# thegenemyers/FASTGA

Measured on NVIDIA H100. Metric: Gbp aligned/sec (genome x genome), higher is better.
Workload: dtype int32

## Files before the change

fastga_b200/csrc/api.cu:

```cuda
#include "common.cuh"
#include "handles.h"
#include <vector>
#include <algorithm>
#include <string.h>
#include <chrono>

typedef unsigned long long u64;

static inline long long now_us()
{ return std::chrono::duration_cast<std::chrono::microseconds>(std::chrono::steady_clock::now().time_since_epoch()).count(); }

extern "C" {
int fgb_kmer_sort_range_device(void *d_a, void *d_b, long long n, unsigned plo, unsigned phi,
                               void *d_tmp, long long tmp_bytes, int *result_in_b, void *stream);
int fgb_sort128_bits_device(void *d_a, void *d_b, long long n, int bit_lo, int bit_hi,
                            void *d_tmp, long long tmp_bytes, int *result_in_b, void *stream);
int fgb_sort128_device(void *d_a, void *d_b, long long n, int byte_lo, int byte_hi,
                       void *d_tmp, long long tmp_bytes, int *result_in_b, void *stream);
long long fgb_sort128_tmp_bytes(long long n);
int fgb_sort_seeds64_device(void *d_a, void *d_b, long long n, int bit_lo, int bit_hi,
                            void *d_tmp, long long tmp_bytes, unsigned long long *d_flag, void *stream);
int fgb_stage_genome_device(const void *d_bps, const long long *d_boff, const long long *d_clen,
                            const long long *d_woff, int ncontig, long long total_words,
                            void *d_seq, void *d_rseq, void *stream);
int fgb_syncmer_count_device(const void *d_seq, const long long *d_clen, const long long *d_woff,
                             const int *d_crank, const int *d_tile_contig, const int *d_tile_start,
                             int ntiles, unsigned *d_tile_count, unsigned long long *d_buck1024,
                             unsigned long long *d_total, void *d_tmp, long long tmp_bytes,
                             unsigned plo, unsigned phi, void *stream);
int fgb_syncmer_emit_device(const void *d_seq, const long long *d_clen, const long long *d_woff,
                            const int *d_crank, const int *d_tile_contig, const int *d_tile_start,
                            int ntiles, unsigned *d_tile_offset, void *d_records, unsigned plo,
                            unsigned phi, void *stream);
int fgb_kix_index_device(const void *d_tab, long long n, unsigned *d_pstart, unsigned char *d_adj, void *stream);
int fgb_ktab_export_device(const void *d_tab, long long n, int pbytes, int cbytes,
                           const long long *d_part_first, int nparts, void *d_out, void *stream);
int fgb_ktab_import_device(const void *d_ent, long long n, int pbytes, int cbytes,
                           const long long *d_index, void *d_tab, void *stream);
int fgb_sc_tile();
int fgb_owner_count_device(const void *d_seeds, long long n, int p_ic, int ic_bits, const int *d_owner, int nrc,
                           int world, unsigned long long *d_cnt, void *stream);
int fgb_owner_scatter_device(const void *d_seeds, long long n, int p_ic, int ic_bits, const int *d_owner, int nrc,
                             int world, unsigned long long *d_base, void *d_out, void *stream);
int fgb_kmer_bins_device(const void *d_tab, long long n, int binshift, unsigned *d_bins, void *stream);
int fgb_self_merge_device(const void *d_T, long long n, const unsigned *d_pstart, int freq,
                          int anti_bits, int band_bits, int jc_bits, int ic_bits,
                          long long amxpos, void *d_seeds, long long capacity,
                          unsigned long long *d_counters, unsigned long long *h_nseeds,
                          unsigned long long *h_sumlen, void *stream);
int fgb_forward_view_device(const void *d_T, long long n, void *d_out, long long *h_nfwd, void *stream);
int fgb_merge_device(const void *d_T1, long long n1, const void *d_T2, long long n2, const unsigned *d_pstart2,
                     const unsigned char *d_adj2, int freq, int anti_bits, int band_bits, int jc_bits, int ic_bits,
                     long long amxpos, long long bmxpos, void *d_seeds, long long capacity,
                     unsigned long long *d_counters, unsigned long long *h_nseeds,
                     unsigned long long *h_sumlen, void *stream);
}

static fgb_timings g_timings;

struct stage_timer
{ cudaEvent_t a, b; cudaStream_t st; float *dst;
  stage_timer(float *d, cudaStream_t s) : st(s), dst(d)
    { cudaEventCreate(&a); cudaEventCreate(&b); cudaEventRecord(a,st); }
  ~stage_timer()
    { cudaEventRecord(b,st); cudaEventSynchronize(b);
      float ms = 0; cudaEventElapsedTime(&ms,a,b); *dst += ms;
      cudaEventDestroy(a); cudaEventDestroy(b);
    }
};

void fgb_timing_add(int which, float ms)
{ if (which == 0) g_timings.triples_ms += ms;
  else if (which == 1) { g_timings.extend_ms += ms; g_timings.extend_launches += 1; }
  else if (which == 3) { g_timings.merge_ms += ms; g_timings.merge_launches += 1; }
  else g_timings.d2h_ms += ms;
}

void fgb_count_launch(int n) { g_timings.launches += n; }


#include <map>
#include <unordered_map>
#include <mutex>

static std::multimap<size_t,void *> g_free;
static std::unordered_map<void *,size_t> g_live;
static std::mutex g_mem_lock;

static size_t size_class(size_t b)
{ if (b < 4096) return 4096;
  size_t p = 4096;
  while (p < b) p <<= 1;
  size_t step = p >> 4;
  return ((b + step - 1) / step) * step;
}

cudaError_t fgb_dmalloc(void **p, size_t bytes, cudaStream_t st)
{ (void) st;
  size_t c = size_class(bytes);
  std::lock_guard<std::mutex> g(g_mem_lock);
  auto it = g_free.lower_bound(c);
  if (it != g_free.end() && it->first <= c + (c >> 2))
    { *p = it->second;
      g_live[*p] = it->first;
      g_free.erase(it);
      return cudaSuccess;
    }
  cudaError_t e = cudaMalloc(p,c);
  if (e != cudaSuccess)
    { cudaGetLastError();
      for (auto &kv : g_free) cudaFree(kv.second);
      g_free.clear();
      e = cudaMalloc(p,c);
      if (e != cudaSuccess) return e;
    }
  g_live[*p] = c;
  return cudaSuccess;
}

void fgb_dfree(void *p, cudaStream_t st)
{ (void) st;
  if (p == NULL) return;
  std::lock_guard<std::mutex> g(g_mem_lock);
  auto it = g_live.find(p);
  if (it == g_live.end()) { cudaFree(p); return; }
  g_free.insert(std::make_pair(it->second,p));
  g_live.erase(it);
}

extern "C" void fgb_release_cache()
{ std::lock_guard<std::mutex> g(g_mem_lock);
  for (auto &kv : g_free) cudaFree(kv.second);
  g_free.clear();
}

extern "C" void fgb_timings_reset() { memset(&g_timings,0,sizeof(g_timings)); }
extern "C" void fgb_timings_get(fgb_timings *out) { *out = g_timings; }


static const long long *g_sort_len;
static int LSORT(const void *l, const void *r)
{ int x = *((const int *) l), y = *((const int *) r);
  return (int) (g_sort_len[y] - g_sort_len[x]);
}

extern "C" int fgb_genome_create(const unsigned char *bps, long long bps_bytes, int ncontig,
                                 const long long *clen, const long long *boff, int want_revcomp,
                                 fgb_genome **out, void *stream)
{ cudaStream_t st = (cudaStream_t) stream;
  if (ncontig <= 0 || ncontig > 0x7fff) return FGB_ERR_LIMIT;
  fgb_genome *g = new fgb_genome();
  g->ncontig = ncontig;
  g->clen.assign(clen,clen+ncontig);
  g->boff.assign(boff,boff+ncontig);
  g->woff.resize(ncontig+1);
  g->seqtot = 0; g->maxlen = 0;
  long long w = 2;
  for (int c = 0; c < ncontig; c++)
    { if (clen[c] >= 0x7fffffffll) { delete g; return FGB_ERR_LIMIT; }
      g->woff[c] = w;
      w += ((clen[c] + 31) >> 5) + 2;
      w = (w + 1) & ~1ll;
      g->seqtot += clen[c];
      if (clen[c] > g->maxlen) g->maxlen = clen[c];
    }
  g->woff[ncontig] = w;
  g->total_words = w;

  g->perm.resize(ncontig); g->crank.resize(ncontig);
  for (int c = 0; c < ncontig; c++) g->perm[c] = c;
  g_sort_len = clen;
  qsort(g->perm.data(),ncontig,sizeof(int),LSORT);
  for (int c = 0; c < ncontig; c++) g->crank[g->perm[c]] = c;

  unsigned char *d_bps = NULL;
  long long *d_boff = NULL;
  CUDA_TRY(fgb_dmalloc((void **) &d_bps,bps_bytes + 16,st));
  CUDA_TRY(fgb_dmalloc((void **) &d_boff,sizeof(long long)*ncontig,st));
  CUDA_TRY(fgb_dmalloc((void **) &g->d_clen,sizeof(long long)*ncontig,st));
  CUDA_TRY(fgb_dmalloc((void **) &g->d_woff,sizeof(long long)*(ncontig+1),st));
  CUDA_TRY(fgb_dmalloc((void **) &g->d_crank,sizeof(int)*ncontig,st));
  CUDA_TRY(fgb_dmalloc((void **) &g->d_perm,sizeof(int)*ncontig,st));
  CUDA_TRY(fgb_dmalloc((void **) &g->d_seq,sizeof(u64)*(w + 1024),st));
  if (want_revcomp) CUDA_TRY(fgb_dmalloc((void **) &g->d_rseq,sizeof(u64)*(w + 1024),st));
  { stage_timer t(&g_timings.h2d_ms,st);
    CUDA_TRY(cudaMemcpyAsync(d_bps,bps,bps_bytes,cudaMemcpyHostToDevice,st));
    CUDA_TRY(cudaMemcpyAsync(d_boff,boff,sizeof(long long)*ncontig,cudaMemcpyHostToDevice,st));
    CUDA_TRY(cudaMemcpyAsync(g->d_clen,clen,sizeof(long long)*ncontig,cudaMemcpyHostToDevice,st));
    CUDA_TRY(cudaMemcpyAsync(g->d_woff,g->woff.data(),sizeof(long long)*(ncontig+1),cudaMemcpyHostToDevice,st));
    CUDA_TRY(cudaMemcpyAsync(g->d_crank,g->crank.data(),sizeof(int)*ncontig,cudaMemcpyHostToDevice,st));
    CUDA_TRY(cudaMemcpyAsync(g->d_perm,g->perm.data(),sizeof(int)*ncontig,cudaMemcpyHostToDevice,st));
  }
  g->h2d_bytes = bps_bytes + (long long) ncontig*(3*8+2*4) + 8;
  int rc;
  { stage_timer t(&g_timings.stage_ms,st);
    rc = fgb_stage_genome_device(d_bps,d_boff,g->d_clen,g->d_woff,ncontig,w,g->d_seq,g->d_rseq,st);
  }
  CUDA_TRY(cudaStreamSynchronize(st));
  fgb_dfree(d_bps,st); fgb_dfree(d_boff,st);
  if (rc) { delete g; return rc; }
  *out = g;
  return FGB_OK;
}

extern "C" void fgb_genome_free(fgb_genome *g)
{ cudaStream_t st = 0;
  if (!g) return;
  fgb_dfree(g->d_clen,st); fgb_dfree(g->d_woff,st); fgb_dfree(g->d_crank,st); fgb_dfree(g->d_perm,st);
  fgb_dfree(g->d_seq,st); fgb_dfree(g->d_rseq,st);
  delete g;
}

extern "C" int fgb_genome_perm(const fgb_genome *g, int *perm_out)
{ memcpy(perm_out,g->perm.data(),sizeof(int)*g->ncontig); return FGB_OK; }

extern "C" int fgb_genome_download(const fgb_genome *g, int rev, unsigned long long *words,
                                   long long *woff_out)
{ const u64 *src = rev ? g->d_rseq : g->d_seq;
  if (src == NULL) return FGB_ERR_ARG;
  CUDA_TRY(cudaMemcpy(words,src,sizeof(u64)*g->total_words,cudaMemcpyDeviceToHost));
  memcpy(woff_out,g->woff.data(),sizeof(long long)*(g->ncontig+1));
  return FGB_OK;
}
extern "C" long long fgb_genome_words(const fgb_genome *g) { return g->total_words; }


extern "C" void fgb_gix_free(fgb_gix *x)
{ cudaStream_t st = 0;
  if (!x) return;
  fgb_dfree(x->d_tab,st); fgb_dfree(x->d_pstart,st); fgb_dfree(x->d_adj,st);
  delete x;
}

static void gix_bytes(const fgb_genome *g, fgb_gix *x)
{ long long cum;
  x->post_bytes = 0;
  for (cum = 1; cum < g->maxlen; cum *= 256) x->post_bytes += 1;
  x->cont_bytes = 0;
  for (cum = 1; cum < 2ll*g->ncontig; cum *= 256) x->cont_bytes += 1;
}


#define GIX_FWD_ONLY 0x80000000u
#define GIX_NO_INDEX 0x40000000u

static int gix_build_range(const fgb_genome *g, unsigned plo, unsigned phi, fgb_gix **out, void *stream);

struct gix_scope
{ fgb_gix *x;
  explicit gix_scope(fgb_gix *p) : x(p) {}
  fgb_gix *release() { fgb_gix *p = x; x = NULL; return p; }
  ~gix_scope() { if (x != NULL) fgb_gix_free(x); }
};
struct blk_scope
{ std::vector<void **> slots;
  template<class T> void own(T *&p) { slots.push_back((void **) &p); }
  ~blk_scope() { for (void **s : slots) if (*s != NULL) { fgb_dfree(*s,0); *s = NULL; } }
};

extern "C" int fgb_gix_build(const fgb_genome *g, fgb_gix **out, void *stream)
{ return gix_build_range(g,0u,1u << 24,out,stream); }

extern "C" int fgb_gix_build_forward(const fgb_genome *g, fgb_gix **out, void *stream)
{ return gix_build_range(g,0u,(1u << 24) | GIX_FWD_ONLY,out,stream); }

extern "C" int fgb_gix_build_range(const fgb_genome *g, unsigned plo, unsigned phi, fgb_gix **out, void *stream)
{ if (plo > phi || phi > (1u << 24)) return FGB_ERR_ARG;
  return gix_build_range(g,plo,phi,out,stream);
}

static int gix_scan(const fgb_genome *g, const unsigned char *mask, unsigned plo, unsigned phi_flags,
                    rec128 **d_recs, long long *n_out, long long *nrev, unsigned long long *buck1024, cudaStream_t st)
{ int T = fgb_sc_tile();
  std::vector<int> tc, ts;
  for (int c = 0; c < g->ncontig; c++)
    if (g->clen[c] >= 12 && g->boff[c] >= 0 && (mask == NULL || mask[c]))
      for (long long t0 = 0; t0 + 12 <= g->clen[c]; t0 += T)
        { tc.push_back(c); ts.push_back((int) t0); }
  int ntiles = (int) tc.size();
  int *d_tc = NULL, *d_ts = NULL; unsigned *d_cnt = NULL;
  u64 *d_buck = NULL, *d_total = NULL; void *d_tmp = NULL;
  rec128 *d_a = NULL;
  long long tmpb = fgb_dev_scan_tmp_bytes(ntiles);
  int rc = FGB_OK;
  u64 total = 0, rdropped = 0;
#define GS_TRY(call) do { if ((call) != cudaSuccess) { rc = FGB_ERR_CUDA; goto done; } } while (0)
  GS_TRY(fgb_dmalloc((void **) &d_tc,sizeof(int)*(ntiles+1),st));
  GS_TRY(fgb_dmalloc((void **) &d_ts,sizeof(int)*(ntiles+1),st));
  GS_TRY(fgb_dmalloc((void **) &d_cnt,sizeof(unsigned)*(ntiles+1),st));
  GS_TRY(fgb_dmalloc((void **) &d_buck,8*1025,st));
  GS_TRY(fgb_dmalloc((void **) &d_total,8,st));
  GS_TRY(fgb_dmalloc((void **) &d_tmp,tmpb,st));
  GS_TRY(cudaMemcpyAsync(d_tc,tc.data(),sizeof(int)*ntiles,cudaMemcpyHostToDevice,st));
  GS_TRY(cudaMemcpyAsync(d_ts,ts.data(),sizeof(int)*ntiles,cudaMemcpyHostToDevice,st));
  { stage_timer t(&g_timings.scan_ms,st);
    rc = fgb_syncmer_count_device(g->d_seq,g->d_clen,g->d_woff,g->d_crank,d_tc,d_ts,ntiles,d_cnt,
                                  d_buck,d_total,d_tmp,tmpb,plo,phi_flags,st);
    if (rc) goto done;
    GS_TRY(cudaMemcpyAsync(&total,d_total,8,cudaMemcpyDeviceToHost,st));
    if (buck1024) GS_TRY(cudaMemcpyAsync(buck1024,d_buck,8*1024,cudaMemcpyDeviceToHost,st));
    GS_TRY(cudaMemcpyAsync(&rdropped,d_buck + 1024,8,cudaMemcpyDeviceToHost,st));
    GS_TRY(cudaStreamSynchronize(st));
  }
  if (total >= 0xfffffff0ull) { rc = FGB_ERR_LIMIT; goto done; }
  GS_TRY(fgb_dmalloc((void **) &d_a,sizeof(rec128)*(total+1),st));
  { stage_timer t(&g_timings.scan_ms,st);
    rc = fgb_syncmer_emit_device(g->d_seq,g->d_clen,g->d_woff,g->d_crank,d_tc,d_ts,ntiles,d_cnt,d_a,plo,phi_flags,st);
  }
  if (rc == FGB_OK && cudaStreamSynchronize(st) != cudaSuccess) rc = FGB_ERR_CUDA;
done:
#undef GS_TRY
  fgb_dfree(d_tc,st); fgb_dfree(d_ts,st); fgb_dfree(d_cnt,st); fgb_dfree(d_buck,st); fgb_dfree(d_total,st); fgb_dfree(d_tmp,st);
  if (rc) { fgb_dfree(d_a,st); return rc; }
  *d_recs = d_a; *n_out = (long long) total; *nrev = (long long) rdropped;
  return FGB_OK;
}

static int gix_finish(fgb_gix *x, rec128 *d_a, long long n, unsigned plo, unsigned phi, cudaStream_t st, bool index = true)
{ rec128 *d_b = NULL; void *d_stmp = NULL;
  long long stmpb = fgb_sort128_tmp_bytes(n);
  int rc = FGB_OK, inb = 0;
  x->n = n;
  if (fgb_dmalloc((void **) &d_b,sizeof(rec128)*(n+1),st) != cudaSuccess ||
      fgb_dmalloc((void **) &d_stmp,stmpb,st) != cudaSuccess ||
      (index && fgb_dmalloc((void **) &x->d_pstart,sizeof(unsigned)*((1<<24)+1+8),st) != cudaSuccess) ||
      (index && fgb_dmalloc((void **) &x->d_adj,(size_t) n + 32,st) != cudaSuccess))
    rc = FGB_ERR_CUDA;
  if (!rc)
    { stage_timer t(&g_timings.ksort_ms,st);
      rc = fgb_kmer_sort_range_device(d_a,d_b,n,plo,phi,d_stmp,stmpb,&inb,st);
    }
  if (!rc)
    { x->d_tab = inb ? d_b : d_a;
      if (inb) d_b = NULL; else d_a = NULL;
      if (index)
        { stage_timer t(&g_timings.index_ms,st);
          rc = fgb_kix_index_device(x->d_tab,n,x->d_pstart,x->d_adj,st);
        }
    }
  if (!rc && cudaStreamSynchronize(st) != cudaSuccess) rc = FGB_ERR_CUDA;
  fgb_dfree(d_a,st); fgb_dfree(d_b,st); fgb_dfree(d_stmp,st);
  return rc;
}

static int gix_build_range(const fgb_genome *g, unsigned plo, unsigned phi_flags, fgb_gix **out, void *stream)
{ cudaStream_t st = (cudaStream_t) stream;
  const bool index = !(phi_flags & GIX_NO_INDEX);
  phi_flags &= ~GIX_NO_INDEX;
  const unsigned phi = phi_flags & ~GIX_FWD_ONLY;
  fgb_gix *x = new fgb_gix();
  gix_bytes(g,x);
  x->ncontig = g->ncontig;
  x->fwd_only = (phi_flags & GIX_FWD_ONLY) ? 1 : 0;
  rec128 *d_a = NULL; long long n = 0, nrev = 0;
  int rc = gix_scan(g,NULL,plo,phi_flags,&d_a,&n,&nrev,x->buck1024,st);
  if (!rc) { x->n_both = n + nrev; rc = gix_finish(x,d_a,n,plo,phi,st,index); }
  if (rc) { fgb_gix_free(x); return rc; }
  *out = x;
  return FGB_OK;
}


extern "C" int fgb_device_alloc(long long bytes, void **out, void *stream)
{ CUDA_TRY(fgb_dmalloc(out,(size_t) (bytes > 0 ? bytes : 16),(cudaStream_t) stream)); return FGB_OK; }
extern "C" void fgb_device_free(void *p) { fgb_dfree(p,0); }

extern "C" int fgb_kmers_scan(const fgb_genome *g, const unsigned char *mask, int fwd_only,
                              void **d_recs, long long *n, void *stream)
{ rec128 *d = NULL; long long nrev = 0;
  int rc = gix_scan(g,mask,0u,(1u << 24) | (fwd_only ? GIX_FWD_ONLY : 0u),&d,n,&nrev,NULL,(cudaStream_t) stream);
  if (rc) return rc;
  *d_recs = d;
  return FGB_OK;
}

extern "C" int fgb_records_group_by_top_byte(void *d_recs, long long n, void *d_out, long long *bounds257,
                                             void *stream)
{ cudaStream_t st = (cudaStream_t) stream;
  for (int b = 0; b <= 256; b++) bounds257[b] = 0;
  if (n <= 0) return FGB_OK;
  void *d_tmp = NULL; unsigned *d_bins = NULL;
  long long tmpb = fgb_sort128_tmp_bytes(n);
  int rc = FGB_OK, inb = 0;
  std::vector<unsigned> bins(65537);
  if (fgb_dmalloc(&d_tmp,tmpb,st) != cudaSuccess || fgb_dmalloc((void **) &d_bins,sizeof(unsigned)*65537,st) != cudaSuccess)
    rc = FGB_ERR_CUDA;
  if (!rc) rc = fgb_sort128_device(d_recs,d_out,n,15,16,d_tmp,tmpb,&inb,st);
  if (!rc && !inb && cudaMemcpyAsync(d_out,d_recs,sizeof(rec128)*n,cudaMemcpyDeviceToDevice,st) != cudaSuccess) rc = FGB_ERR_CUDA;
  if (!rc) rc = fgb_kmer_bins_device(d_out,n,56,d_bins,st);
  if (!rc && (cudaMemcpyAsync(bins.data(),d_bins,sizeof(unsigned)*65537,cudaMemcpyDeviceToHost,st) != cudaSuccess ||
              cudaStreamSynchronize(st) != cudaSuccess)) rc = FGB_ERR_CUDA;
  fgb_dfree(d_tmp,st); fgb_dfree(d_bins,st);
  if (rc) return rc;
  for (int b = 0; b <= 256; b++) bounds257[b] = bins[b];
  return FGB_OK;
}

extern "C" int fgb_gix_from_records(const void *d_recs, long long n, unsigned plo, unsigned phi, int fwd_only,
                                    int post_bytes, int cont_bytes, int ncontig, fgb_gix **out, void *stream)
{ cudaStream_t st = (cudaStream_t) stream;
  if (n < 0 || n >= 0xfffffff0ll || plo >= phi || phi > (1u << 24)) return FGB_ERR_ARG;
  fgb_gix *x = new fgb_gix();
  x->n_both = n; x->post_bytes = post_bytes; x->cont_bytes = cont_bytes; x->ncontig = ncontig;
  x->fwd_only = fwd_only ? 1 : 0;
  rec128 *d_a = NULL;
  int rc = FGB_OK;
  if (fgb_dmalloc((void **) &d_a,sizeof(rec128)*(n+1),st) != cudaSuccess) rc = FGB_ERR_CUDA;
  if (!rc && n > 0 && cudaMemcpyAsync(d_a,d_recs,sizeof(rec128)*n,cudaMemcpyDeviceToDevice,st) != cudaSuccess) rc = FGB_ERR_CUDA;
  if (!rc) rc = gix_finish(x,d_a,n,plo,phi,st); else fgb_dfree(d_a,st);
  if (rc) { fgb_gix_free(x); return rc; }
  *out = x;
  return FGB_OK;
}

extern "C" long long fgb_gix_size(const fgb_gix *x) { return x->n; }

extern "C" int fgb_gix_copy_table(const fgb_gix *x, void *d_dst, void *stream)
{ CUDA_TRY(cudaMemcpyAsync(d_dst,x->d_tab,sizeof(rec128)*x->n,cudaMemcpyDeviceToDevice,(cudaStream_t) stream));
  CUDA_TRY(cudaStreamSynchronize((cudaStream_t) stream));
  return FGB_OK;
}

extern "C" int fgb_gix_from_device(const void *d_tab, long long n, int post_bytes, int cont_bytes,
                                   int ncontig, fgb_gix **out, void *stream)
{ cudaStream_t st = (cudaStream_t) stream;
  if (n >= 0xfffffff0ll) return FGB_ERR_LIMIT;
  fgb_gix *x = new fgb_gix();
  gix_scope own(x);
  x->n = n; x->n_both = n; x->post_bytes = post_bytes; x->cont_bytes = cont_bytes; x->ncontig = ncontig;
  CUDA_TRY(fgb_dmalloc((void **) &x->d_tab,sizeof(rec128)*(n+1),st));
  CUDA_TRY(fgb_dmalloc((void **) &x->d_pstart,sizeof(unsigned)*((1<<24)+1+8),st));
  CUDA_TRY(fgb_dmalloc((void **) &x->d_adj,(size_t) x->n + 32,st));
  CUDA_TRY(cudaMemcpyAsync(x->d_tab,d_tab,sizeof(rec128)*n,cudaMemcpyDeviceToDevice,st));
  int rc;
  { stage_timer t(&g_timings.index_ms,st);
    rc = fgb_kix_index_device(x->d_tab,n,x->d_pstart,x->d_adj,st);
  }
  CUDA_TRY(cudaStreamSynchronize(st));
  if (rc) return rc;
  *out = own.release();
  return FGB_OK;
}
extern "C" int fgb_gix_post_bytes(const fgb_gix *x) { return x->post_bytes; }
extern "C" int fgb_gix_cont_bytes(const fgb_gix *x) { return x->cont_bytes; }

extern "C" int fgb_gix_download(const fgb_gix *x, void *tab , unsigned *pstart ,
                                unsigned long long *buck1024)
{ if (tab) CUDA_TRY(cudaMemcpy(tab,x->d_tab,sizeof(rec128)*x->n,cudaMemcpyDeviceToHost));
  if (pstart) CUDA_TRY(cudaMemcpy(pstart,x->d_pstart,sizeof(unsigned)*((1<<24)+1),cudaMemcpyDeviceToHost));
  if (buck1024) memcpy(buck1024,x->buck1024,8*1024);
  return FGB_OK;
}

extern "C" int fgb_gix_upload(const void *tab, long long n, int post_bytes, int cont_bytes,
                              int ncontig, fgb_gix **out, void *stream)
{ cudaStream_t st = (cudaStream_t) stream;
  if (n >= 0xfffffff0ll) return FGB_ERR_LIMIT;
  fgb_gix *x = new fgb_gix();
  gix_scope own(x);
  x->n = n; x->n_both = n; x->post_bytes = post_bytes; x->cont_bytes = cont_bytes; x->ncontig = ncontig;
  CUDA_TRY(fgb_dmalloc((void **) &x->d_tab,sizeof(rec128)*(n+1),st));
  CUDA_TRY(fgb_dmalloc((void **) &x->d_pstart,sizeof(unsigned)*((1<<24)+1+8),st));
  CUDA_TRY(fgb_dmalloc((void **) &x->d_adj,(size_t) x->n + 32,st));
  CUDA_TRY(cudaMemcpyAsync(x->d_tab,tab,sizeof(rec128)*n,cudaMemcpyHostToDevice,st));
  int rc = fgb_kix_index_device(x->d_tab,n,x->d_pstart,x->d_adj,st);
  CUDA_TRY(cudaStreamSynchronize(st));
  if (rc) return rc;
  *out = own.release();
  return FGB_OK;
}

extern "C" int fgb_gix_import_ktab(const unsigned char *entries, long long n, int post_bytes,
                                   int cont_bytes, const long long *index, int ncontig,
                                   fgb_gix **out, void *stream)
{ cudaStream_t st = (cudaStream_t) stream;
  if (n >= 0xfffffff0ll || post_bytes > 4 || cont_bytes > 2) return FGB_ERR_LIMIT;
  fgb_gix *x = new fgb_gix();
  gix_scope own(x);
  x->n = n; x->n_both = n; x->post_bytes = post_bytes; x->cont_bytes = cont_bytes; x->ncontig = ncontig;
  long long E = 9 + post_bytes + cont_bytes;
  unsigned char *d_ent = NULL; long long *d_index = NULL;
  blk_scope B; B.own(d_ent); B.own(d_index);
  CUDA_TRY(fgb_dmalloc((void **) &d_ent,E*n + 16,st));
  CUDA_TRY(fgb_dmalloc((void **) &d_index,8ll<<24,st));
  CUDA_TRY(fgb_dmalloc((void **) &x->d_tab,sizeof(rec128)*(n+1),st));
  CUDA_TRY(fgb_dmalloc((void **) &x->d_pstart,sizeof(unsigned)*((1<<24)+1+8),st));
  CUDA_TRY(fgb_dmalloc((void **) &x->d_adj,(size_t) x->n + 32,st));
  CUDA_TRY(cudaMemcpyAsync(d_ent,entries,E*n,cudaMemcpyHostToDevice,st));
  CUDA_TRY(cudaMemcpyAsync(d_index,index,8ll<<24,cudaMemcpyHostToDevice,st));
  int rc = fgb_ktab_import_device(d_ent,n,post_bytes,cont_bytes,d_index,x->d_tab,st);
  if (!rc) rc = fgb_kix_index_device(x->d_tab,n,x->d_pstart,x->d_adj,st);
  CUDA_TRY(cudaStreamSynchronize(st));
  if (rc) return rc;
  *out = own.release();
  return FGB_OK;
}

extern "C" int fgb_gix_export_ktab(const fgb_gix *x, const long long *part_first, int nparts,
                                   unsigned char *out, void *stream)
{ cudaStream_t st = (cudaStream_t) stream;
  long long E = 9 + x->post_bytes + x->cont_bytes;
  unsigned char *d_out = NULL; long long *d_pf = NULL;
  blk_scope B; B.own(d_out); B.own(d_pf);
  CUDA_TRY(fgb_dmalloc((void **) &d_out,E*x->n + 16,st));
  CUDA_TRY(fgb_dmalloc((void **) &d_pf,8*(nparts+1),st));
  CUDA_TRY(cudaMemcpyAsync(d_pf,part_first,8*nparts,cudaMemcpyHostToDevice,st));
  int rc = fgb_ktab_export_device(x->d_tab,x->n,x->post_bytes,x->cont_bytes,d_pf,nparts,d_out,st);
  if (!rc) CUDA_TRY(cudaMemcpyAsync(out,d_out,E*x->n,cudaMemcpyDeviceToHost,st));
  CUDA_TRY(cudaStreamSynchronize(st));
  return rc;
}


static int bitlen(long long v) { int b = 0; while (v > 0) { b += 1; v >>= 1; } return b; }

extern "C" void fgb_seeds_free(fgb_seeds *s)
{ cudaStream_t st = 0;
  if (!s) return;
  fgb_dfree(s->d_rec,st);
  delete s;
}

static int seeds_find_impl(const fgb_gix *x1, const fgb_gix *x2, long long amxpos,
                           long long bmxpos, int freq, bool self, fgb_seeds **out, void *stream);

extern "C" int fgb_seeds_find(const fgb_gix *x1, const fgb_gix *x2, long long amxpos,
                              long long bmxpos, int freq, fgb_seeds **out, void *stream)
{ return seeds_find_impl(x1,x2,amxpos,bmxpos,freq,false,out,stream); }

extern "C" int fgb_seeds_find_self(const fgb_gix *x, long long amxpos, int freq, fgb_seeds **out, void *stream)
{ return seeds_find_impl(x,x,amxpos,amxpos,freq,true,out,stream); }

struct seed_bits { int anti, band, jc, ic, key; };

static int seed_layout_of(const fgb_gix *x1, const fgb_gix *x2, long long amxpos, long long bmxpos, seed_bits *L)
{ L->anti = bitlen(amxpos + bmxpos);
  L->band = L->anti > 6 ? L->anti - 6 : 1;
  L->jc   = bitlen(x2->ncontig > 1 ? x2->ncontig-1 : 1);
  L->ic   = bitlen(x1->ncontig > 1 ? x1->ncontig-1 : 1);
  L->key  = 12 + L->anti + L->band + L->jc + L->ic + 1;
  return L->key > 128 ? FGB_ERR_LIMIT : FGB_OK;
}

static int seeds_merge_impl(const fgb_gix *x1, const fgb_gix *x2, long long amxpos, long long bmxpos, int freq,
                            bool self, const seed_bits &L, rec128 **d_out, long long *nseeds_out,
                            long long *sumlen_out, long long *n1m_out, cudaStream_t st)
{ if (self && x1->fwd_only) return FGB_ERR_ARG;
  u64 *d_counters = NULL; rec128 *d_fwd = NULL, *d_a = NULL;
  int rc = FGB_OK;
  u64 nseeds = 0, sumlen = 0;
  const rec128 *t1 = x1->d_tab; long long n1 = x1->n;
#define SF_TRY(call) do { if ((call) != cudaSuccess) { rc = FGB_ERR_CUDA; goto done; } } while (0)
  SF_TRY(fgb_dmalloc((void **) &d_counters,16,st));
  if (!self && !x1->fwd_only && n1 > 0)
    { SF_TRY(fgb_dmalloc((void **) &d_fwd,sizeof(rec128)*(n1+1),st));
      if ((rc = fgb_forward_view_device(x1->d_tab,n1,d_fwd,&n1,st))) goto done;
      t1 = d_fwd;
    }
  { long long cap = (self ? 2*x1->n : 2*n1 + (n1 >> 1)) + 1024;
    for (int attempt = 0; ; attempt++)
      { SF_TRY(fgb_dmalloc((void **) &d_a,sizeof(rec128)*(cap+1),st));
        if (self)
          rc = fgb_self_merge_device(x1->d_tab,x1->n,x1->d_pstart,freq,L.anti,L.band,L.jc,L.ic,amxpos,
                                     d_a,cap,d_counters,&nseeds,&sumlen,st);
        else
          rc = fgb_merge_device(t1,n1,x2->d_tab,x2->n,x2->d_pstart,x2->d_adj,freq,L.anti,L.band,L.jc,L.ic,
                                amxpos,bmxpos,d_a,cap,d_counters,&nseeds,&sumlen,st);
        if (rc == FGB_OK) break;
        fgb_dfree(d_a,st); d_a = NULL;
        if (rc != FGB_ERR_OVERFLOW || attempt > 0) goto done;
        cap = (long long) nseeds + 1024;
        g_timings.merge_ms = 0; g_timings.merge_launches = 0;
      }
  }
  if (nseeds >= 0xfffffff0ull) rc = FGB_ERR_LIMIT;
done:
#undef SF_TRY
  fgb_dfree(d_counters,st); fgb_dfree(d_fwd,st);
  if (rc) { fgb_dfree(d_a,st); return rc; }
  *d_out = d_a; *nseeds_out = (long long) nseeds; *sumlen_out = (long long) sumlen; *n1m_out = n1;
  return FGB_OK;
}

static int seeds_sort_impl(rec128 *d_a, long long n, const seed_bits &L, long long amxpos, long long bmxpos,
                           bool self, long long sumlen, long long n1m, fgb_seeds **out, cudaStream_t st)
{ rec128 *d_b = NULL; void *d_tmp = NULL;
  fgb_seeds *s = new fgb_seeds();
  s->self_mode = self ? 1 : 0;
  s->anti_bits = L.anti; s->band_bits = L.band; s->jc_bits = L.jc; s->ic_bits = L.ic;
  s->amxpos = amxpos; s->bmxpos = bmxpos;
  s->n = n; s->sumlen = sumlen; s->n1_merged = n1m;
  long long tmpb = fgb_sort128_tmp_bytes(n);
  int rc = FGB_OK, inb = 0;
  const char *wide_env = getenv("FGB_SEED_SORT_WIDE");
  const bool narrow = L.key <= 64 && !(wide_env != NULL && atoi(wide_env) != 0);
  u64 hiflag = 0, *d_hiflag = NULL;
  if (fgb_dmalloc((void **) &d_b,sizeof(rec128)*(n+1),st) != cudaSuccess ||
      fgb_dmalloc((void **) &d_tmp,tmpb + 8,st) != cudaSuccess) rc = FGB_ERR_CUDA;
  if (!rc)
    { stage_timer t(&g_timings.ssort_ms,st);
      if (narrow)
        { d_hiflag = (u64 *) ((char *) d_tmp + tmpb);
          rc = fgb_sort_seeds64_device(d_a,d_b,n,6,L.key,d_tmp,tmpb,d_hiflag,st);
        }
      else
        rc = fgb_sort128_bits_device(d_a,d_b,n,6,L.key,d_tmp,tmpb,&inb,st);
    }
  if (!rc && d_hiflag && cudaMemcpyAsync(&hiflag,d_hiflag,8,cudaMemcpyDeviceToHost,st) != cudaSuccess) rc = FGB_ERR_CUDA;
  if (!rc && cudaStreamSynchronize(st) != cudaSuccess) rc = FGB_ERR_CUDA;
  if (!rc && hiflag) rc = FGB_ERR_ARG;
  if (!rc)
    { s->d_rec = inb ? d_b : d_a;
      if (inb) d_b = NULL; else d_a = NULL;
    }
  fgb_dfree(d_a,st); fgb_dfree(d_b,st); fgb_dfree(d_tmp,st);
  if (rc) { delete s; return rc; }
  *out = s;
  return FGB_OK;
}

static int seeds_find_impl(const fgb_gix *x1, const fgb_gix *x2, long long amxpos,
                           long long bmxpos, int freq, bool self, fgb_seeds **out, void *stream)
{ cudaStream_t st = (cudaStream_t) stream;
  seed_bits L;
  int rc = seed_layout_of(x1,x2,amxpos,bmxpos,&L);
  if (rc) return rc;
  rec128 *d_a = NULL; long long n = 0, sumlen = 0, n1m = 0;
  if ((rc = seeds_merge_impl(x1,x2,amxpos,bmxpos,freq,self,L,&d_a,&n,&sumlen,&n1m,st))) return rc;
  return seeds_sort_impl(d_a,n,L,amxpos,bmxpos,self,sumlen,n1m,out,st);
}


extern "C" int fgb_seeds_merge(const fgb_gix *x1, const fgb_gix *x2, long long amxpos, long long bmxpos, int freq,
                               void **d_seeds, long long *n, int *bits, long long *info, void *stream)
{ seed_bits L;
  int rc = seed_layout_of(x1,x2,amxpos,bmxpos,&L);
  if (rc) return rc;
  rec128 *d_a = NULL; long long sumlen = 0, n1m = 0;
  if ((rc = seeds_merge_impl(x1,x2,amxpos,bmxpos,freq,false,L,&d_a,n,&sumlen,&n1m,(cudaStream_t) stream))) return rc;
  *d_seeds = d_a;
  bits[0] = L.anti; bits[1] = L.band; bits[2] = L.jc; bits[3] = L.ic;
  if (info) { info[0] = sumlen; info[1] = n1m; }
  return FGB_OK;
}

extern "C" int fgb_seeds_group_by_owner(const void *d_seeds, long long n, const int *bits, const int *owner,
                                        int nrank_contigs, int world, void *d_out, long long *bounds,
                                        void *stream)
{ cudaStream_t st = (cudaStream_t) stream;
  if (world < 1 || world > 64) return FGB_ERR_ARG;
  for (int w = 0; w <= world; w++) bounds[w] = 0;
  if (n <= 0) return FGB_OK;
  int *d_owner = NULL; u64 *d_cnt = NULL;
  int rc = FGB_OK;
  u64 cnt[64], base[65];
  const int p_ic = 12 + bits[0] + bits[1] + bits[2];
  if (fgb_dmalloc((void **) &d_owner,sizeof(int)*(size_t) nrank_contigs,st) != cudaSuccess ||
      fgb_dmalloc((void **) &d_cnt,8*64*2,st) != cudaSuccess) rc = FGB_ERR_CUDA;
  if (!rc && (cudaMemcpyAsync(d_owner,owner,sizeof(int)*(size_t) nrank_contigs,cudaMemcpyHostToDevice,st) != cudaSuccess ||
              cudaMemsetAsync(d_cnt,0,8*64*2,st) != cudaSuccess)) rc = FGB_ERR_CUDA;
  if (!rc) rc = fgb_owner_count_device(d_seeds,n,p_ic,bits[3],d_owner,nrank_contigs,world,d_cnt,st);
  if (!rc && (cudaMemcpyAsync(cnt,d_cnt,8*64,cudaMemcpyDeviceToHost,st) != cudaSuccess ||
              cudaStreamSynchronize(st) != cudaSuccess)) rc = FGB_ERR_CUDA;
  if (!rc)
    { base[0] = 0;
      for (int w = 0; w < world; w++) base[w+1] = base[w] + cnt[w];
      if (cudaMemcpyAsync(d_cnt + 64,base,8*64,cudaMemcpyHostToDevice,st) != cudaSuccess) rc = FGB_ERR_CUDA;
    }
  if (!rc) rc = fgb_owner_scatter_device(d_seeds,n,p_ic,bits[3],d_owner,nrank_contigs,world,d_cnt + 64,d_out,st);
  if (!rc && cudaStreamSynchronize(st) != cudaSuccess) rc = FGB_ERR_CUDA;
  fgb_dfree(d_owner,st); fgb_dfree(d_cnt,st);
  if (rc) return rc;
  for (int w = 0; w <= world; w++) bounds[w] = (long long) base[w];
  return FGB_OK;
}

extern "C" int fgb_records_group_by_owner(const void *d_recs, long long n, const int *owner256, int world,
                                          void *d_out, long long *bounds, void *stream)
{ cudaStream_t st = (cudaStream_t) stream;
  if (world < 1 || world > 64) return FGB_ERR_ARG;
  for (int w = 0; w <= world; w++) bounds[w] = 0;
  if (n <= 0) return FGB_OK;
  int *d_owner = NULL; u64 *d_cnt = NULL;
  int rc = FGB_OK;
  u64 cnt[64], base[65];
  if (fgb_dmalloc((void **) &d_owner,sizeof(int)*256,st) != cudaSuccess ||
      fgb_dmalloc((void **) &d_cnt,8*64*2,st) != cudaSuccess) rc = FGB_ERR_CUDA;
  if (!rc && (cudaMemcpyAsync(d_owner,owner256,sizeof(int)*256,cudaMemcpyHostToDevice,st) != cudaSuccess ||
              cudaMemsetAsync(d_cnt,0,8*64*2,st) != cudaSuccess)) rc = FGB_ERR_CUDA;
  if (!rc) rc = fgb_owner_count_device(d_recs,n,120,8,d_owner,256,world,d_cnt,st);
  if (!rc && (cudaMemcpyAsync(cnt,d_cnt,8*64,cudaMemcpyDeviceToHost,st) != cudaSuccess ||
              cudaStreamSynchronize(st) != cudaSuccess)) rc = FGB_ERR_CUDA;
  if (!rc)
    { base[0] = 0;
      for (int w = 0; w < world; w++) base[w+1] = base[w] + cnt[w];
      if (cudaMemcpyAsync(d_cnt + 64,base,8*64,cudaMemcpyHostToDevice,st) != cudaSuccess) rc = FGB_ERR_CUDA;
    }
  if (!rc) rc = fgb_owner_scatter_device(d_recs,n,120,8,d_owner,256,world,d_cnt + 64,d_out,st);
  if (!rc && cudaStreamSynchronize(st) != cudaSuccess) rc = FGB_ERR_CUDA;
  fgb_dfree(d_owner,st); fgb_dfree(d_cnt,st);
  if (rc) return rc;
  for (int w = 0; w <= world; w++) bounds[w] = (long long) base[w];
  return FGB_OK;
}

extern "C" int fgb_seeds_from_records(const void *d_recs, long long n, const int *bits, long long amxpos,
                                      long long bmxpos, long long sumlen, fgb_seeds **out, void *stream)
{ cudaStream_t st = (cudaStream_t) stream;
  if (n < 0 || n >= 0xfffffff0ll) return FGB_ERR_LIMIT;
  seed_bits L;
  L.anti = bits[0]; L.band = bits[1]; L.jc = bits[2]; L.ic = bits[3];
  L.key = 12 + L.anti + L.band + L.jc + L.ic + 1;
  if (L.key > 128) return FGB_ERR_LIMIT;
  rec128 *d_a = NULL;
  CUDA_TRY(fgb_dmalloc((void **) &d_a,sizeof(rec128)*(n+1),st));
  if (n > 0 && cudaMemcpyAsync(d_a,d_recs,sizeof(rec128)*n,cudaMemcpyDeviceToDevice,st) != cudaSuccess)
    { fgb_dfree(d_a,st); return FGB_ERR_CUDA; }
  return seeds_sort_impl(d_a,n,L,amxpos,bmxpos,false,sumlen,0,out,st);
}

extern "C" long long fgb_seeds_size(const fgb_seeds *s) { return s->n; }
extern "C" long long fgb_seeds_sumlen(const fgb_seeds *s) { return s->sumlen; }
extern "C" int fgb_seeds_layout(const fgb_seeds *s, int *bits )
{ bits[0] = s->anti_bits; bits[1] = s->band_bits; bits[2] = s->jc_bits; bits[3] = s->ic_bits; return FGB_OK; }
extern "C" int fgb_seeds_download(const fgb_seeds *s, void *rec)
{ CUDA_TRY(cudaMemcpy(rec,s->d_rec,sizeof(rec128)*s->n,cudaMemcpyDeviceToHost)); return FGB_OK; }

extern "C" int fgb_sort128_host(void *recs, long long n, int byte_lo, int byte_hi, void *stream)
{ cudaStream_t st = (cudaStream_t) stream;
  rec128 *d_a = NULL, *d_b = NULL; void *d_tmp = NULL;
  long long tmpb = fgb_sort128_tmp_bytes(n);
  CUDA_TRY(fgb_dmalloc((void **) &d_a,sizeof(rec128)*(n+1),st));
  CUDA_TRY(fgb_dmalloc((void **) &d_b,sizeof(rec128)*(n+1),st));
  CUDA_TRY(fgb_dmalloc((void **) &d_tmp,tmpb,st));
  CUDA_TRY(cudaMemcpyAsync(d_a,recs,sizeof(rec128)*n,cudaMemcpyHostToDevice,st));
  int inb = 0;
  int rc = fgb_sort128_device(d_a,d_b,n,byte_lo,byte_hi,d_tmp,tmpb,&inb,st);
  if (!rc) CUDA_TRY(cudaMemcpyAsync(recs,inb ? d_b : d_a,sizeof(rec128)*n,cudaMemcpyDeviceToHost,st));
  CUDA_TRY(cudaStreamSynchronize(st));
  fgb_dfree(d_a,st); fgb_dfree(d_b,st); fgb_dfree(d_tmp,st);
  return rc;
}

extern "C" int fgb_device_ready()
{ int n = 0;
  if (cudaGetDeviceCount(&n) != cudaSuccess || n == 0) return 0;
  return 1;
}


struct fgb_overlaps;
struct fgb_alns;
extern "C" {
int fgb_extend(const fgb_seeds *S, const fgb_genome *A, const fgb_genome *B, int chain_break,
               int chain_min, int align_min, double align_rate, const short *tables, int ave_path,
               int tspace, fgb_overlaps **out, void *stream);
int fgb_align_spec(double ave_corr, const float *freq, short *tables, int *ave_path);
void fgb_overlaps_free(fgb_overlaps *o);
long long fgb_overlaps_bytes(const fgb_overlaps *o);
void fgb_overlaps_counters(const fgb_overlaps *o, unsigned long long *out);
int fgb_filter(const fgb_overlaps *O, const int *perm1, const int *perm2, int jc_bits, int ic_bits,
               int do_filter, fgb_alns **out);
}

struct fgb_run_stats
{ long long nkmers1, nkmers2, nseeds, sumlen, nhits, nla, nwaves, ncells, nraw, h2d_bytes, d2h_bytes,
            nseg, nwork, warp_cycles, wave_cycles, extract_cycles,
            us_gix, us_seeds, us_extend, us_filter, nkmers1_fwd,
            slow_cycles, slow_waves, paired_waves, pairings; };

extern "C" int fgb_align_tables(const fgb_genome *A, const fgb_genome *B, const fgb_gix *x1,
                                const fgb_gix *x2, const float *freqA,
                                int freq, int chain_break, int chain_min, int align_min,
                                double align_rate, fgb_alns **out, fgb_run_stats *stats, void *stream);

static int align_tables_impl(const fgb_genome *A, const fgb_genome *B, fgb_gix *x1, fgb_gix *x2, bool own,
                             const float *freqA, int freq, int chain_break, int chain_min, int align_min,
                             double align_rate, fgb_alns **out, fgb_run_stats *stats, void *stream);

extern "C" int fgb_align_resident(const fgb_genome *A, const fgb_genome *B, const float *freqA,
                                  int freq, int chain_break, int chain_min, int align_min,
                                  double align_rate, fgb_alns **out, fgb_run_stats *stats, void *stream)
{ fgb_gix *x1 = NULL, *x2 = NULL;
  int rc;
  long long t0 = now_us();
  if ((rc = gix_build_range(A,0u,(1u << 24) | GIX_FWD_ONLY | GIX_NO_INDEX,&x1,stream))) return rc;
  if ((rc = fgb_gix_build(B,&x2,stream))) { fgb_gix_free(x1); return rc; }
  long long t1 = now_us();
  rc = align_tables_impl(A,B,x1,x2,true,freqA,freq,chain_break,chain_min,align_min,align_rate,out,stats,stream);
  if (stats) stats->us_gix = t1 - t0;
  return rc;
}

extern "C" int fgb_align_tables(const fgb_genome *A, const fgb_genome *B, const fgb_gix *x1,
                                const fgb_gix *x2, const float *freqA,
                                int freq, int chain_break, int chain_min, int align_min,
                                double align_rate, fgb_alns **out, fgb_run_stats *stats, void *stream)
{ return align_tables_impl(A,B,(fgb_gix *) x1,(fgb_gix *) x2,false,freqA,freq,chain_break,chain_min,align_min,
                           align_rate,out,stats,stream);
}

static int align_tables_impl(const fgb_genome *A, const fgb_genome *B, fgb_gix *x1, fgb_gix *x2, bool own,
                             const float *freqA, int freq, int chain_break, int chain_min, int align_min,
                             double align_rate, fgb_alns **out, fgb_run_stats *stats, void *stream)
{ fgb_seeds *sd = NULL; fgb_overlaps *ov = NULL;
  int rc;
  long long t0 = now_us(), t1 = t0, t2, t3, t4;
  const long long n1 = x1->n_both, n2 = x2->n;
  { seed_bits L;
    rec128 *d_a = NULL; long long n = 0, sumlen = 0, n1m = 0;
    rc = seed_layout_of(x1,x2,A->maxlen,B->maxlen,&L);
    if (!rc) rc = seeds_merge_impl(x1,x2,A->maxlen,B->maxlen,freq,false,L,&d_a,&n,&sumlen,&n1m,(cudaStream_t) stream);
    if (own) { fgb_gix_free(x1); fgb_gix_free(x2); }
    if (!rc) rc = seeds_sort_impl(d_a,n,L,A->maxlen,B->maxlen,false,sumlen,n1m,&sd,(cudaStream_t) stream);
  }
  if (rc) return rc;
  const long long n1f = sd->n1_merged;
  t2 = now_us();
  short *tables = (short *) malloc(65536*sizeof(short));
  int ave = 0;
  fgb_align_spec(1.-align_rate,freqA,tables,&ave);
  rc = fgb_extend(sd,A,B,chain_break,chain_min,align_min,align_rate,tables,ave,100,&ov,stream);
  free(tables);
  t3 = now_us();
  long long nseeds = sd->n, sumlen = sd->sumlen;
  int jb = sd->jc_bits, ib = sd->ic_bits;
  fgb_seeds_free(sd);
  if (rc) return rc;
  rc = fgb_filter(ov,A->perm.data(),B->perm.data(),jb,ib,1,out);
  t4 = now_us();
  if (stats)
    { stats->us_gix = t1-t0; stats->us_seeds = t2-t1; stats->us_extend = t3-t2; stats->us_filter = t4-t3; unsigned long long c[16];
      fgb_overlaps_counters(ov,c);
      stats->nkmers1 = n1; stats->nkmers2 = n2; stats->nseeds = nseeds; stats->sumlen = sumlen;
      stats->nkmers1_fwd = n1f;
      stats->nhits = (long long) c[0]; stats->nla = (long long) c[1]; stats->nwaves = (long long) c[2];
      stats->ncells = (long long) c[3]; stats->nraw = 0;
      stats->nseg = (long long) c[5]; stats->nwork = (long long) c[6];
      stats->warp_cycles = (long long) c[8]; stats->wave_cycles = (long long) c[9];
      stats->extract_cycles = (long long) c[10];
      stats->slow_cycles = (long long) ((c[15] >> 40) << 12); stats->slow_waves = (long long) ((c[15] >> 16) & 0xffffff);
      stats->paired_waves = (long long) c[11]; stats->pairings = (long long) c[12];
      stats->h2d_bytes = A->h2d_bytes + B->h2d_bytes + 65536*2;
      stats->d2h_bytes = fgb_overlaps_bytes(ov) + 16 + 8*1024*2 + 64;
    }
  fgb_overlaps_free(ov);
  return rc;
}

extern "C" int fgb_fastga_self(const unsigned char *bps, long long nb, int nc, const long long *clen,
                               const long long *boff, const float *freq4,
                               int freq, int chain_break, int chain_min, int align_min, double align_rate,
                               fgb_alns **out, fgb_run_stats *stats, void *stream)
{ fgb_genome *A = NULL; fgb_gix *x = NULL; fgb_seeds *sd = NULL; fgb_overlaps *ov = NULL;
  int rc;
  if ((rc = fgb_genome_create(bps,nb,nc,clen,boff,1,&A,stream))) return rc;
  if ((rc = fgb_gix_build(A,&x,stream))) { fgb_genome_free(A); return rc; }
  rc = fgb_seeds_find_self(x,A->maxlen,freq,&sd,stream);
  long long n1 = x->n;
  fgb_gix_free(x);
  if (rc) { fgb_genome_free(A); return rc; }
  short *tables = (short *) malloc(65536*sizeof(short));
  int ave = 0;
  fgb_align_spec(1.-align_rate,freq4,tables,&ave);
  rc = fgb_extend(sd,A,A,chain_break,chain_min,align_min,align_rate,tables,ave,100,&ov,stream);
  free(tables);
  long long nseeds = sd->n, sumlen = sd->sumlen;
  int jb = sd->jc_bits, ib = sd->ic_bits;
  fgb_seeds_free(sd);
  if (rc) { fgb_genome_free(A); return rc; }
  rc = fgb_filter(ov,A->perm.data(),A->perm.data(),jb,ib,1,out);
  if (stats)
    { memset(stats,0,sizeof(*stats));
      unsigned long long c[16];
      fgb_overlaps_counters(ov,c);
      stats->nkmers1 = stats->nkmers2 = n1; stats->nseeds = nseeds; stats->sumlen = sumlen;
      stats->nhits = (long long) c[0]; stats->nla = (long long) c[1]; stats->nwaves = (long long) c[2];
      stats->ncells = (long long) c[3];
    }
  fgb_overlaps_free(ov);
  fgb_genome_free(A);
  return rc;
}

extern "C" int fgb_fastga(const unsigned char *bpsA, long long nbA, int ncA, const long long *clenA,
                          const long long *boffA, const float *freqA,
                          const unsigned char *bpsB, long long nbB, int ncB, const long long *clenB,
                          const long long *boffB,
                          int freq, int chain_break, int chain_min, int align_min, double align_rate,
                          fgb_alns **out, fgb_run_stats *stats, void *stream)
{ fgb_genome *A = NULL, *B = NULL;
  int rc;
  if ((rc = fgb_genome_create(bpsA,nbA,ncA,clenA,boffA,1,&A,stream))) return rc;
  if ((rc = fgb_genome_create(bpsB,nbB,ncB,clenB,boffB,0,&B,stream))) { fgb_genome_free(A); return rc; }
  rc = fgb_align_resident(A,B,freqA,freq,chain_break,chain_min,align_min,align_rate,out,stats,stream);
  fgb_genome_free(A); fgb_genome_free(B);
  return rc;
}
```

fastga_b200/csrc/gix.cu:

```cuda
#include "common.cuh"

static const unsigned char h_TMap[256] =
  { 0xff,0xd4,0xf5,0xfd,0xe4,0xad,0x21,0xa5,0xed,0x64,0xbf,0xa9,0xf3,0x70,0xd6,0xf0,
    0xca,0x89,0xcb,0xc9,0x82,0x9d,0x13,0x79,0x0a,0x0f,0x25,0x19,0x3e,0x47,0xa3,0xa8,
    0xf9,0x5e,0xe8,0xa1,0xb0,0x71,0x1d,0x8c,0xde,0x69,0xe7,0x7c,0x56,0x3f,0x90,0xa4,
    0xeb,0x45,0x59,0xf1,0x97,0x4c,0x08,0xa0,0xb8,0x4a,0x86,0xc8,0xcd,0x98,0x7d,0xfc,
    0xef,0x4d,0x83,0x7e,0xdc,0x66,0x2b,0x8e,0xe0,0xa7,0xd0,0xa2,0x88,0x5f,0x7f,0xd9,
    0x9b,0x78,0xd1,0x8b,0xc3,0x8f,0x2d,0xe6,0x18,0x27,0x2c,0x24,0x94,0xb7,0xce,0xbd,
    0x0d,0x04,0x1c,0x09,0x16,0x23,0x00,0x1e,0x1a,0x29,0x2e,0x15,0x01,0x10,0x2a,0x20,
    0xbe,0x31,0x43,0x58,0xc2,0xaa,0x1f,0xe5,0xc5,0x9e,0xcf,0xc6,0x68,0xb2,0x80,0xf4,
    0xf8,0x53,0xb6,0x93,0x76,0x37,0x11,0x40,0xda,0x51,0xba,0x46,0x42,0x30,0x60,0x6d,
    0x5c,0x39,0x9f,0x48,0x6c,0x62,0x28,0x67,0x06,0x12,0x26,0x0e,0x33,0x50,0xa6,0x63,
    0xdd,0x3b,0xab,0x4b,0x72,0x5b,0x22,0x6f,0xb4,0x61,0x92,0x99,0x36,0x38,0x65,0xac,
    0x4f,0x2f,0x32,0x44,0x54,0x3c,0x03,0x5d,0x73,0x3a,0x77,0x84,0x8d,0x4e,0x49,0xd2,
    0xfb,0x91,0x6a,0xcc,0x8a,0x35,0x02,0x55,0x7a,0x34,0x96,0x3d,0xd3,0x41,0x85,0xf2,
    0xb1,0x75,0xc4,0xb5,0xbb,0xb3,0x1b,0xd5,0x07,0x05,0x17,0x0b,0x7b,0xd7,0xdf,0xea,
    0xe3,0x57,0xc0,0x95,0x9c,0x6e,0x14,0xae,0xb9,0x6b,0xc1,0x81,0x87,0x74,0xd8,0xe2,
    0xec,0x52,0xbc,0xe9,0xe1,0xdb,0x0c,0xf7,0xaf,0x5a,0x9a,0xc7,0xfa,0xf6,0xee,0xfe };

__constant__ unsigned char c_TN[256];
__constant__ unsigned char c_TC[256];

static int tables_ready = 0;

static int init_tables()
{ if (tables_ready) return FGB_OK;
  unsigned char tn[256], tc[256];
  for (int x = 0; x < 256; x++)
    { int b0 = x & 3, b1 = (x>>2) & 3, b2 = (x>>4) & 3, b3 = (x>>6) & 3;
      int fwd = (b0<<6) | (b1<<4) | (b2<<2) | b3;
      int rc  = ((3-b3)<<6) | ((3-b2)<<4) | ((3-b1)<<2) | (3-b0);
      tn[x] = h_TMap[fwd];
      tc[x] = h_TMap[rc];
    }
  CUDA_TRY(cudaMemcpyToSymbol(c_TN,tn,256));
  CUDA_TRY(cudaMemcpyToSymbol(c_TC,tc,256));
  tables_ready = 1;
  return FGB_OK;
}

typedef unsigned long long u64;


static __device__ __forceinline__ u64 bases64(const u64 *__restrict__ w, long long nw, long long boff)
{ long long q = boff >> 5;
  int s = (int) (boff & 31) << 1;
  u64 a = (q >= 0 && q < nw) ? w[q] : 0ull;
  if (s == 0) return a;
  u64 b = (q+1 >= 0 && q+1 < nw) ? w[q+1] : 0ull;
  return (a >> s) | (b << (64-s));
}

static __device__ __forceinline__ u64 rev2(u64 x)
{ x = __brevll(x);
  return ((x & 0x5555555555555555ull) << 1) | ((x >> 1) & 0x5555555555555555ull);
}


__global__ void stage_contigs_kernel(const unsigned char *__restrict__ bps,
                                     const long long *__restrict__ boff,
                                     const long long *__restrict__ clen,
                                     const long long *__restrict__ woff, int ncontig,
                                     u64 *__restrict__ seq, long long total_words)
{ long long g = (long long) blockIdx.x * blockDim.x + threadIdx.x;
  if (g >= total_words) return;
  int lo = 0, hi = ncontig-1;
  while (lo < hi)
    { int m = (lo+hi+1) >> 1;
      if (woff[m] <= g) lo = m; else hi = m-1;
    }
  long long q = g - woff[lo];
  long long nbytes = (clen[lo]+3) >> 2;
  long long b0 = q*8;
  u64 v = 0;
  if (boff[lo] >= 0 && q >= 0)
    { const unsigned char *p = bps + boff[lo];
      for (int i = 0; i < 8; i++)
        if (b0+i < nbytes)
          v |= (u64) p[b0+i] << (8*i);
      long long lim = clen[lo] - q*32;
      if (lim < 32) v &= (lim <= 0) ? 0ull : ((1ull << (2*lim)) - 1);
    }
  seq[g] = v;
}

__global__ void revcomp_contigs_kernel(const u64 *__restrict__ seq, const long long *__restrict__ clen,
                                       const long long *__restrict__ woff, int ncontig,
                                       u64 *__restrict__ rseq, long long total_words)
{ long long g = (long long) blockIdx.x * blockDim.x + threadIdx.x;
  if (g >= total_words) return;
  int lo = 0, hi = ncontig-1;
  while (lo < hi)
    { int m = (lo+hi+1) >> 1;
      if (woff[m] <= g) lo = m; else hi = m-1;
    }
  long long q = g - woff[lo];
  long long L = clen[lo];
  long long nw = (lo+1 < ncontig ? woff[lo+1] : total_words) - woff[lo];
  if (q < 0) { rseq[g] = 0; return; }
  u64 e = bases64(seq + woff[lo],nw,L - 32 - 32*q);
  u64 v = ~rev2(e);
  long long lim = L - q*32;
  if (lim < 32) v &= (lim <= 0) ? 0ull : ((1ull << (2*lim)) - 1);
  rseq[g] = v;
}


#define SC_THREADS 256
#define SC_PPT     16
#define SC_TILE    (SC_THREADS*SC_PPT)
#define SC_WORDS   (SC_TILE/32 + 3)

static __device__ __forceinline__ u64 sm_bases64(const u64 *sw, int boff)
{ int q = boff >> 5, s = (boff & 31) << 1;
  u64 a = sw[q];
  if (s == 0) return a;
  return (a >> s) | (sw[q+1] << (64-s));
}


static __device__ __forceinline__ unsigned syncmer_mask(u64 E, const unsigned char *tn,
                                                        const unsigned char *tc)
{ unsigned hn[SC_PPT+8], hc[SC_PPT+8];
#pragma unroll
  for (int i = 0; i < SC_PPT+8; i++)
    { unsigned x = (unsigned) (E >> (2*i)) & 0xff;
      hn[i] = tn[x];
      hc[i] = tc[x];
    }
  unsigned mz[SC_PPT+4];
#pragma unroll
  for (int i = 0; i < SC_PPT+4; i++)
    { unsigned mn = (hn[i] << 8) | hn[i+4];
      unsigned mc = hc[i] | (hc[i+4] << 8);
      mz[i] = mn < mc ? mn : mc;
    }
  unsigned sel = 0;
#pragma unroll
  for (int i = 0; i < SC_PPT; i++)
    { unsigned m = min(min(min(mz[i],mz[i+1]),min(mz[i+2],mz[i+3])),mz[i+4]);
      if (mz[i] == m || mz[i+4] == m) sel |= 1u << i;
    }
  return sel;
}

template<int EMIT> __global__ void __launch_bounds__(SC_THREADS)
syncmer_kernel(const u64 *__restrict__ seq, const long long *__restrict__ clen,
               const long long *__restrict__ woff, const int *__restrict__ crank,
               const int *__restrict__ tile_contig, const int *__restrict__ tile_start,
               unsigned *__restrict__ tile_count,
               unsigned long long *__restrict__ buck1024,
               rec128 *__restrict__ out, unsigned plo, unsigned phi_flags)
{ __shared__ u64 sw[SC_WORDS+1];
  __shared__ unsigned char tn[256], tc[256];
  __shared__ unsigned wsum[SC_THREADS/32];
  __shared__ unsigned hist[1024];

  const unsigned phi = phi_flags & 0x7fffffffu;
  const bool fwd_only = (phi_flags >> 31) != 0;
  int tid = threadIdx.x;
  int c   = tile_contig[blockIdx.x];
  int t0  = tile_start[blockIdx.x];
  long long L  = clen[c];
  const u64 *w = seq + woff[c];
  long long nw = (L + 31) >> 5;

  tn[tid] = c_TN[tid];
  tc[tid] = c_TC[tid];
  if (EMIT == 0)
    for (int i = tid; i < 1024; i += SC_THREADS) hist[i] = 0;
  for (int i = tid; i < SC_WORDS+1; i += SC_THREADS)
    { long long gw = (t0 >> 5) - 1 + i;
      sw[i] = (gw >= 0 && gw < nw) ? w[gw] : 0ull;
    }
  __syncthreads();

  int p = t0 + tid*SC_PPT;
  int sb = 32 + tid*SC_PPT;
  unsigned sel = 0;
  if ((long long) p + 12 <= L)
    { sel = syncmer_mask(sm_bases64(sw,sb),tn,tc);
      long long lastok = L - 12 - p;
      if (lastok < SC_PPT-1) sel &= (2u << lastok) - 1;
    }

  unsigned fmask = sel, rmask = sel;
  { long long fl = L - 40 - p;
    if (fl < 0) fmask = 0; else if (fl < SC_PPT-1) fmask &= (2u << fl) - 1;
    int rl = 28 - p;
    if (rl > 0) rmask = (rl >= SC_PPT) ? 0 : (rmask & ~((1u << rl) - 1));
  }
  if (plo != 0 || phi != (1u << 24))
    { unsigned m = fmask | rmask;
      while (m)
        { int i = __ffs(m)-1;
          m &= m-1;
          if (fmask >> i & 1)
            { unsigned pf = (unsigned) (rev2(sm_bases64(sw,sb+i)) >> 40);
              if (pf < plo || pf >= phi) fmask &= ~(1u << i);
            }
          if (rmask >> i & 1)
            { u64 e0 = sm_bases64(sw,sb+i-28), e1 = sm_bases64(sw,sb+i+4) & 0xffffull;
              unsigned pr = (unsigned) ((~((e1 << 48) | (e0 >> 16))) >> 40);
              if (pr < plo || pr >= phi) rmask &= ~(1u << i);
            }
        }
    }
  unsigned rdropped = 0;
  if (fwd_only) { rdropped = __popc(rmask); rmask = 0; }
  unsigned cnt = __popc(fmask) + __popc(rmask);

  int lane = tid & 31, wp = tid >> 5;
  unsigned inc = cnt;
#pragma unroll
  for (int o = 1; o < 32; o <<= 1)
    { unsigned t = __shfl_up_sync(0xffffffffu,inc,o);
      if (lane >= o) inc += t;
    }
  if (lane == 31) wsum[wp] = inc;
  __syncthreads();
  unsigned pre = 0, tot = 0;
  for (int i = 0; i < SC_THREADS/32; i++)
    { if (i < wp) pre += wsum[i];
      tot += wsum[i];
    }

  if (EMIT == 0)
    {
      unsigned m = sel;
      while (m)
        { int i = __ffs(m)-1;
          m &= m-1;
          u64 f = sm_bases64(sw,sb+i);
          unsigned fb = (unsigned) (rev2(f) >> 54);
          u64 r = sm_bases64(sw,sb+i+7);
          unsigned rb = (unsigned) ((~r) & 0x3ff);
          unsigned rr = 0;
#pragma unroll
          for (int k = 0; k < 5; k++)
            rr |= ((rb >> (2*k)) & 3) << (2*k);
          atomicAdd(&hist[fb],1u);
          atomicAdd(&hist[rr],1u);
        }
      __syncthreads();
      for (int i = tid; i < 1024; i += SC_THREADS)
        if (hist[i]) atomicAdd(&buck1024[i],(unsigned long long) hist[i]);
      if (fwd_only)
        { rdropped = __reduce_add_sync(0xffffffffu,rdropped);
          if (lane == 0 && rdropped) atomicAdd(&buck1024[1024],(unsigned long long) rdropped);
        }
      if (tid == 0) tile_count[blockIdx.x] = tot;
      return;
    }

  long long o = (long long) tile_count[blockIdx.x] + pre + inc - cnt;
  unsigned cr = (unsigned) crank[c];
  unsigned m = fmask | rmask;
  while (m)
    { int i = __ffs(m)-1;
      m &= m-1;
      int j = p + i;
      if (fmask >> i & 1)
        { u64 e0 = sm_bases64(sw,sb+i);
          u64 e1 = sm_bases64(sw,sb+i+32);
          rec128 r;
          r.hi = rev2(e0);
          r.lo = (rev2(e1) & 0xffff000000000000ull) | ((u64) cr << 32) | (unsigned) j;
          st_rec(out + o,r);
          o += 1;
        }
      if (rmask >> i & 1)
        { u64 e0 = sm_bases64(sw,sb+i-28);
          u64 e1 = sm_bases64(sw,sb+i+4) & 0xffffull;
          rec128 r;
          r.hi = ~((e1 << 48) | (e0 >> 16));
          r.lo = ((~e0 & 0xffffull) << 48) | ((u64) (cr | 0x8000u) << 32) | (unsigned) (j+12);
          st_rec(out + o,r);
          o += 1;
        }
    }
}


__global__ void kix_index_kernel(const rec128 *__restrict__ tab, long long n,
                                 unsigned *__restrict__ pstart, unsigned char *__restrict__ adj)
{ long long i = (long long) blockIdx.x * blockDim.x + threadIdx.x;
  if (i > n) return;
  rec128 a, b;
  a.lo = a.hi = b.lo = b.hi = 0;
  if (i > 0) a = ld_rec(tab + i - 1);
  if (i < n) b = ld_rec(tab + i);
  if (i > 0 && i < n)
    { long long plo = (long long) KREC_PREFIX24(a.hi), phi = (long long) KREC_PREFIX24(b.hi);
      for (long long x = plo+1; x <= phi; x++)
        pstart[x] = (unsigned) i;
    }
  int l = 0;
  if (i > 0 && i < n)
    { unsigned long long x = a.hi ^ b.hi;
      if (x) l = __clzll(x) >> 1;
      else
        { unsigned y = (unsigned) ((a.lo ^ b.lo) >> 48);
          l = y ? 32 + ((__clz(y) - 16) >> 1) : 40;
        }
    }
  adj[i] = (unsigned char) l;
}

static __device__ __forceinline__ int krec_lcp(const rec128 &a, const rec128 &b)
{ u64 x = a.hi ^ b.hi;
  if (x) return __clzll(x) >> 1;
  unsigned y = (unsigned) ((a.lo ^ b.lo) >> 48);
  if (y) return 32 + ((__clz(y) - 16) >> 1);
  return 40;
}


__global__ void ktab_export_kernel(const rec128 *__restrict__ tab, long long n, int pbytes,
                                   int cbytes, const long long *__restrict__ part_first, int nparts,
                                   unsigned char *__restrict__ out)
{ long long i = (long long) blockIdx.x * blockDim.x + threadIdx.x;
  if (i >= n) return;
  rec128 r = tab[i];
  int lcp = 0;
  bool first = false;
  for (int p = 0; p < nparts; p++)
    if (part_first[p] == i) first = true;
  if (!first)
    lcp = krec_lcp(tab[i-1],r);
  int E = 9 + pbytes + cbytes;
  unsigned char *o = out + i*E;
  u64 suf = KREC_SUFFIX56(r);
  for (int k = 0; k < 7; k++)
    o[k] = (unsigned char) (suf >> (8*(6-k)));
  o[7] = 0;
  o[8] = (unsigned char) lcp;
  unsigned post = (unsigned) r.lo;
  for (int k = 0; k < pbytes; k++)
    o[9+k] = (unsigned char) (post >> (8*k));
  unsigned cs = (unsigned) (r.lo >> 32) & 0xffff;
  unsigned cv = (cs & 0x7fff) | ((cs >> 15) << (8*cbytes-1));
  for (int k = 0; k < cbytes; k++)
    o[9+pbytes+k] = (unsigned char) (cv >> (8*k));
}


__global__ void ktab_import_kernel(const unsigned char *__restrict__ ent, long long n, int pbytes,
                                   int cbytes, const long long *__restrict__ index ,
                                   rec128 *__restrict__ tab)
{ long long i = (long long) blockIdx.x * blockDim.x + threadIdx.x;
  if (i >= n) return;
  int lo = 0, hi = (1<<24)-1;
  while (lo < hi)
    { int m = (lo+hi) >> 1;
      if (index[m] > i) hi = m; else lo = m+1;
    }
  int E = 9 + pbytes + cbytes;
  const unsigned char *e = ent + i*E;
  u64 suf = 0;
  for (int k = 0; k < 7; k++)
    suf = (suf << 8) | e[k];
  unsigned post = 0;
  for (int k = 0; k < pbytes; k++)
    post |= (unsigned) e[9+k] << (8*k);
  unsigned cv = 0;
  for (int k = 0; k < cbytes; k++)
    cv |= (unsigned) e[9+pbytes+k] << (8*k);
  unsigned sign = cv >> (8*cbytes-1);
  unsigned cs = (cv & ((1u << (8*cbytes-1)) - 1)) | (sign << 15);
  rec128 r;
  r.hi = ((u64) lo << 40) | (suf >> 16);
  r.lo = ((suf & 0xffffull) << 48) | ((u64) cs << 32) | post;
  st_rec(tab + i,r);
}


extern "C" int fgb_sort128_device(void *d_a, void *d_b, long long n, int byte_lo, int byte_hi,
                                  void *d_tmp, long long tmp_bytes, int *result_in_b, void *stream);
extern "C" long long fgb_sort128_tmp_bytes(long long n);

extern "C" int fgb_stage_genome_device(const void *d_bps, const long long *d_boff,
                                       const long long *d_clen, const long long *d_woff,
                                       int ncontig, long long total_words, void *d_seq,
                                       void *d_rseq , void *stream)
{ cudaStream_t st = (cudaStream_t) stream;
  if (total_words <= 0) return FGB_OK;
  int nb = (int) ((total_words + 255) / 256);
  stage_contigs_kernel<<<nb,256,0,st>>>((const unsigned char *) d_bps,d_boff,d_clen,d_woff,ncontig,
                                        (u64 *) d_seq,total_words);
  if (d_rseq != NULL)
    revcomp_contigs_kernel<<<nb,256,0,st>>>((const u64 *) d_seq,d_clen,d_woff,ncontig,
                                            (u64 *) d_rseq,total_words);
  fgb_count_launch(d_rseq != NULL ? 2 : 1);
  CUDA_TRY(cudaGetLastError());
  return FGB_OK;
}


extern "C" int fgb_syncmer_count_device(const void *d_seq, const long long *d_clen,
                                        const long long *d_woff, const int *d_crank,
                                        const int *d_tile_contig, const int *d_tile_start, int ntiles,
                                        unsigned *d_tile_count, unsigned long long *d_buck1024,
                                        unsigned long long *d_total, void *d_tmp, long long tmp_bytes,
                                        unsigned plo, unsigned phi, void *stream)
{ cudaStream_t st = (cudaStream_t) stream;
  int rc = init_tables();
  if (rc) return rc;
  CUDA_TRY(cudaMemsetAsync(d_buck1024,0,1025*8,st));
  if (ntiles > 0)
    syncmer_kernel<0><<<ntiles,SC_THREADS,0,st>>>((const u64 *) d_seq,d_clen,d_woff,d_crank,
                                                   d_tile_contig,d_tile_start,d_tile_count,
                                                   d_buck1024,NULL,plo,phi);
  fgb_count_launch(1);
  CUDA_TRY(cudaGetLastError());
  return fgb_dev_exclusive_scan_u32(d_tile_count,ntiles,d_total,d_tmp,tmp_bytes,st);
}

extern "C" int fgb_syncmer_emit_device(const void *d_seq, const long long *d_clen,
                                       const long long *d_woff, const int *d_crank,
                                       const int *d_tile_contig, const int *d_tile_start, int ntiles,
                                       unsigned *d_tile_offset, void *d_records, unsigned plo,
                                       unsigned phi, void *stream)
{ cudaStream_t st = (cudaStream_t) stream;
  if (ntiles > 0)
    syncmer_kernel<1><<<ntiles,SC_THREADS,0,st>>>((const u64 *) d_seq,d_clen,d_woff,d_crank,
                                                   d_tile_contig,d_tile_start,d_tile_offset,
                                                   NULL,(rec128 *) d_records,plo,phi);
  fgb_count_launch(1);
  CUDA_TRY(cudaGetLastError());
  return FGB_OK;
}

__global__ void kix_ends_kernel(const rec128 *__restrict__ tab, long long n, unsigned *__restrict__ pstart)
{ long long x = (long long) blockIdx.x * blockDim.x + threadIdx.x;
  if (x > (1ll << 24)) return;
  if (n == 0) { pstart[x] = 0; return; }
  long long p0 = (long long) KREC_PREFIX24(tab[0].hi), pl = (long long) KREC_PREFIX24(tab[n-1].hi);
  if (x <= p0) pstart[x] = 0;
  else if (x > pl) pstart[x] = (unsigned) n;
}

extern "C" int fgb_kix_index_device(const void *d_tab, long long n, unsigned *d_pstart, unsigned char *d_adj,
                                    void *stream)
{ cudaStream_t st = (cudaStream_t) stream;
  int nb = (int) ((n + 1 + 255) / 256);
  CUDA_TRY(cudaMemsetAsync(d_adj + n,0,32,st));
  kix_index_kernel<<<nb,256,0,st>>>((const rec128 *) d_tab,n,d_pstart,d_adj);
  kix_ends_kernel<<<((1 << 24) + 256)/256,256,0,st>>>((const rec128 *) d_tab,n,d_pstart);
  fgb_count_launch(1);
  CUDA_TRY(cudaGetLastError());
  return FGB_OK;
}

extern "C" int fgb_ktab_export_device(const void *d_tab, long long n, int pbytes, int cbytes,
                                      const long long *d_part_first, int nparts, void *d_out,
                                      void *stream)
{ cudaStream_t st = (cudaStream_t) stream;
  if (n <= 0) return FGB_OK;
  int nb = (int) ((n + 255) / 256);
  ktab_export_kernel<<<nb,256,0,st>>>((const rec128 *) d_tab,n,pbytes,cbytes,d_part_first,nparts,
                                      (unsigned char *) d_out);
  CUDA_TRY(cudaGetLastError());
  return FGB_OK;
}

extern "C" int fgb_ktab_import_device(const void *d_ent, long long n, int pbytes, int cbytes,
                                      const long long *d_index, void *d_tab, void *stream)
{ cudaStream_t st = (cudaStream_t) stream;
  if (n <= 0) return FGB_OK;
  int nb = (int) ((n + 255) / 256);
  ktab_import_kernel<<<nb,256,0,st>>>((const unsigned char *) d_ent,n,pbytes,cbytes,d_index,
                                      (rec128 *) d_tab);
  CUDA_TRY(cudaGetLastError());
  return FGB_OK;
}

extern "C" int fgb_sc_tile() { return SC_TILE; }
```

fastga_b200/csrc/sort128.cu:

```cuda
#include "common.cuh"
#include <stdlib.h>
#include <vector>

#define SORT_THREADS 512
#ifndef SORT_ITEMS
#define SORT_ITEMS   8
#endif
#ifndef SORT_MINBLK
#define SORT_MINBLK  2
#endif
#define SORT_TILE    (SORT_THREADS*SORT_ITEMS)
#define SORT_WARPS   (SORT_THREADS/32)

static __device__ __forceinline__ unsigned warp_incl_scan(unsigned v, int lane)
{
#pragma unroll
  for (int o = 1; o < 32; o <<= 1)
    { unsigned t = __shfl_up_sync(0xffffffffu,v,o);
      if (lane >= o) v += t;
    }
  return v;
}



static __device__ __forceinline__ unsigned match_digit(unsigned d, bool valid)
{ unsigned peers = __ballot_sync(0xffffffffu,valid);
#pragma unroll
  for (int k = 0; k < 8; k++)
    { bool bit = (d >> k) & 1;
      unsigned bk = __ballot_sync(0xffffffffu,bit);
      peers &= bit ? bk : ~bk;
    }
  return peers;
}


#define ST_AGG  (1ull << 62)
#define ST_INC  (2ull << 62)
#define ST_MASK ((1ull << 62) - 1)

__global__ void __launch_bounds__(SORT_THREADS)
sort_ghist_kernel(const rec128 *__restrict__ in, long long n, int dsh , unsigned long long *__restrict__ ghist)
{ __shared__ unsigned h[256];
  int tid = threadIdx.x;
  if (tid < 256) h[tid] = 0;
  __syncthreads();
  const bool one = (dsh >= 64 || dsh <= 56);
  const unsigned long long *half = reinterpret_cast<const unsigned long long *>(in) + (dsh >= 64);
  const int sh = dsh & 63;
  for (long long tile0 = (long long) blockIdx.x * SORT_TILE; tile0 < n; tile0 += (long long) gridDim.x * SORT_TILE)
    {
#pragma unroll
      for (int it = 0; it < SORT_ITEMS; it++)
        { long long idx = tile0 + it*SORT_THREADS + tid;
          bool valid = idx < n;
          unsigned d = 0;
          if (valid) d = one ? (unsigned) ((half[2*idx] >> sh) & 0xff) : rec_dig(ld_rec(in + idx),dsh);
          unsigned peers = match_digit(d,valid);
          if (valid && (tid & 31) == __ffs(peers)-1) atomicAdd(&h[d],__popc(peers));
        }
    }
  __syncthreads();
  if (tid < 256 && h[tid]) atomicAdd(&ghist[tid],(unsigned long long) h[tid]);
}

__global__ void sort_bins_kernel(const unsigned long long *__restrict__ ghist, unsigned long long *__restrict__ binbase,
                                 unsigned long long *__restrict__ nexthist, unsigned *__restrict__ ticket)
{ __shared__ unsigned long long ws[8];
  int tid = threadIdx.x, lane = tid & 31, w = tid >> 5;
  unsigned long long v = ghist[tid], inc = v;
  for (int o = 1; o < 32; o <<= 1)
    { unsigned long long t = __shfl_up_sync(0xffffffffu,inc,o);
      if (lane >= o) inc += t;
    }
  if (lane == 31) ws[w] = inc;
  __syncthreads();
  unsigned long long pre = 0;
  for (int i = 0; i < w; i++) pre += ws[i];
  binbase[tid] = pre + inc - v;
  nexthist[tid] = 0;
  if (tid == 0) *ticket = 0;
}

__global__ void __launch_bounds__(SORT_THREADS,SORT_MINBLK)
sort_onesweep_kernel(const rec128 *__restrict__ in, rec128 *__restrict__ out, long long n, int byte ,
                     int next_byte , const unsigned long long *__restrict__ binbase,
                     unsigned long long *__restrict__ nexthist, unsigned long long *status ,
                     unsigned *__restrict__ ticket)
{ extern __shared__ __align__(16) unsigned char smem_raw[];
  rec128   *tile   = reinterpret_cast<rec128 *>(smem_raw);
  unsigned *wcount = reinterpret_cast<unsigned *>(tile + SORT_TILE);
  unsigned *bexcl  = wcount + SORT_WARPS*256;
  unsigned *nhist  = bexcl + 256;
  unsigned *wtot   = nhist + 256;
  unsigned long long *gbase = reinterpret_cast<unsigned long long *>(wtot + 8);
  __shared__ unsigned tile_s;
  __shared__ __align__(8) unsigned long long tbar;

  int tid = threadIdx.x, lane = tid & 31, w = tid >> 5;
  if (tid == 0)
    { unsigned t = atomicAdd(ticket,1u);
      tile_s = t;
      long long t0 = (long long) t * SORT_TILE, rm = n - t0;
      unsigned nb = (unsigned) (rm < SORT_TILE ? rm : SORT_TILE) * 16u;
      mbar_init(&tbar,1);
      tma_load_1d(tile,in + t0,nb,&tbar);
    }
  for (int i = tid; i < SORT_WARPS*256; i += SORT_THREADS) wcount[i] = 0;
  if (tid < 256) nhist[tid] = 0;
  __syncthreads();
  const unsigned tileid = tile_s;
  long long tile0 = (long long) tileid * SORT_TILE;
  long long rem = n - tile0;
  int cnt = rem < SORT_TILE ? (int) rem : SORT_TILE;

  rec128   r[SORT_ITEMS];
  unsigned rank[SORT_ITEMS];
  int base = w*(32*SORT_ITEMS);
  unsigned *myc = wcount + w*256;
  mbar_wait(&tbar,0);
#pragma unroll
  for (int it = 0; it < SORT_ITEMS; it++)
    { int idx = base + it*32 + lane;
      bool valid = idx < cnt;
      unsigned d = 0;
      if (valid)
        { r[it] = ld_rec(tile + idx);
          d = rec_dig(r[it],byte);
        }
      unsigned peers = match_digit(d,valid);
      int leader = valid ? __ffs(peers)-1 : lane;
      unsigned b = 0;
      if (valid && lane == leader)
        { b = myc[d];
          myc[d] = b + __popc(peers);
        }
      b = __shfl_sync(0xffffffffu,b,leader);
      rank[it] = b + __popc(peers & lanemask_lt());
      if (next_byte >= 0 && valid) atomicAdd(&nhist[rec_dig(r[it],next_byte)],1u);
      __syncwarp();
    }
  __syncthreads();

  unsigned c = 0, inc = 0;
  unsigned long long *mine = status + (unsigned long long) tileid*256 + tid;
  if (tid < 256)
    { unsigned sum = 0;
#pragma unroll
      for (int ww = 0; ww < SORT_WARPS; ww++)
        { unsigned t = wcount[ww*256+tid];
          wcount[ww*256+tid] = sum;
          sum += t;
        }
      c = sum;
      if (tileid == 0)
        atomicExch(mine,ST_INC | c);
      else
        atomicExch(mine,ST_AGG | c);
      inc = warp_incl_scan(c,lane);
      if (lane == 31) wtot[w] = inc;
    }
  __syncthreads();
  if (tid < 256)
    { unsigned pre = 0;
      for (int i = 0; i < w; i++) pre += wtot[i];
      bexcl[tid] = pre + inc - c;
    }
  __syncthreads();

#pragma unroll
  for (int it = 0; it < SORT_ITEMS; it++)
    { int idx = base + it*32 + lane;
      if (idx < cnt)
        { unsigned d = rec_dig(r[it],byte);
          st_rec(tile + (bexcl[d] + myc[d] + rank[it]),r[it]);
        }
    }
  if (tid < 256)
    {
      volatile unsigned long long *stt = status;
      unsigned long long excl = 0;
      for (long long t = (long long) tileid - 1; t >= 0; )
        { unsigned long long v[4];
#pragma unroll
          for (int q = 0; q < 4; q++)
            v[q] = (t - q >= 0) ? stt[(unsigned long long) (t - q)*256 + tid] : ST_INC;
          bool done = false;
#pragma unroll
          for (int q = 0; q < 4; q++)
            { if (done || (v[q] >> 62) == 0) break;
              excl += v[q] & ST_MASK;
              t -= 1;
              if (v[q] & ST_INC) done = true;
            }
          if (done) break;
        }
      if (tileid != 0) atomicExch(mine,ST_INC | (excl + c));
      gbase[tid] = binbase[tid] + excl - bexcl[tid];
      if (next_byte >= 0 && nhist[tid]) atomicAdd(&nexthist[tid],(unsigned long long) nhist[tid]);
    }
  __syncthreads();

  for (int p = tid; p < cnt; p += SORT_THREADS)
    { rec128 v = ld_rec(tile + p);
      unsigned d = rec_dig(v,byte);
      st_rec(out + (gbase[d] + p),v);
    }
}

static const size_t ONESWEEP_SMEM = SORT_TILE*sizeof(rec128) + (SORT_WARPS*256 + 256 + 256 + 8)*sizeof(unsigned)
                                    + 256*sizeof(unsigned long long);

extern "C" long long fgb_sort128_tmp_bytes(long long n)
{ long long ntiles = (n + SORT_TILE - 1) / SORT_TILE;
  if (ntiles < 1) ntiles = 1;
  return 256*ntiles*8 + (3*256 + 16)*8;
}


extern "C" int fgb_sort128_bits_device(void *d_a, void *d_b, long long n, int bit_lo, int bit_hi,
                                       void *d_tmp, long long tmp_bytes, int *result_in_b, void *stream)
{ cudaStream_t st = (cudaStream_t) stream;
  if (n < 0 || bit_lo < 0 || bit_hi > 128 || bit_lo > bit_hi) return FGB_ERR_ARG;
  if (n >= 0xffffffffll) return FGB_ERR_LIMIT;
  *result_in_b = 0;
  if (n <= 1 || bit_lo == bit_hi) return FGB_OK;
  if (tmp_bytes < fgb_sort128_tmp_bytes(n)) return FGB_ERR_ARG;

  int ntiles = (int) ((n + SORT_TILE - 1) / SORT_TILE);
  unsigned long long *status = (unsigned long long *) d_tmp;
  unsigned long long *hist[2] = { status + 256ull*ntiles, status + 256ull*ntiles + 256 };
  unsigned long long *binbase = status + 256ull*ntiles + 512;
  unsigned *ticket = (unsigned *) (binbase + 256);

  static bool attr_set = false;
  if (!attr_set)
    { CUDA_TRY(cudaFuncSetAttribute(sort_onesweep_kernel,cudaFuncAttributeMaxDynamicSharedMemorySize,
                                    (int) ONESWEEP_SMEM));
      attr_set = true;
    }

  rec128 *src = (rec128 *) d_a, *dst = (rec128 *) d_b;
  CUDA_TRY(cudaMemsetAsync(hist[0],0,256*8,st));
  { int nb = ntiles < 1184 ? ntiles : 1184;
    sort_ghist_kernel<<<nb,SORT_THREADS,0,st>>>(src,n,bit_lo,hist[0]);
    fgb_count_launch(1);
  }
  int cur = 0;
  for (int b = bit_lo; b < bit_hi; b += 8)
    { sort_bins_kernel<<<1,256,0,st>>>(hist[cur],binbase,hist[cur^1],ticket);
      CUDA_TRY(cudaMemsetAsync(status,0,256ull*ntiles*8,st));
      sort_onesweep_kernel<<<ntiles,SORT_THREADS,ONESWEEP_SMEM,st>>>(src,dst,n,b,(b+8 < bit_hi) ? b+8 : -1,
                                                                   binbase,hist[cur^1],status,ticket);
      fgb_count_launch(2);
      cur ^= 1;
      rec128 *t = src; src = dst; dst = t;
      *result_in_b ^= 1;
    }
  CUDA_TRY(cudaGetLastError());
  return FGB_OK;
}

extern "C" int fgb_sort128_device(void *d_a, void *d_b, long long n, int byte_lo, int byte_hi,
                                  void *d_tmp, long long tmp_bytes, int *result_in_b, void *stream)
{ if (byte_lo < 0 || byte_hi > 16 || byte_lo > byte_hi) return FGB_ERR_ARG;
  return fgb_sort128_bits_device(d_a,d_b,n,8*byte_lo,8*byte_hi,d_tmp,tmp_bytes,result_in_b,stream);
}


#ifndef SORT64_ITEMS
#define SORT64_ITEMS 16
#endif
static_assert(SORT_THREADS*SORT64_ITEMS >= SORT_TILE, "fgb_sort128_tmp_bytes sizes the look-back status for SORT_TILE");

template <int IW> struct os64_tile
{ static constexpr int ITEMS = (IW == 16) ? SORT_ITEMS : SORT64_ITEMS;
  static constexpr int TILE  = SORT_THREADS*ITEMS;
  static constexpr size_t SMEM = (size_t) TILE*IW + (SORT_WARPS*256 + 256 + 256 + 8)*sizeof(unsigned)
                                 + 256*sizeof(unsigned long long);
};

template <int IW, int OW>
__global__ void __launch_bounds__(SORT_THREADS,SORT_MINBLK)
sort_onesweep64_kernel(const void *__restrict__ in, void *__restrict__ out, long long n, int dsh ,
                       int next_dsh , const unsigned long long *__restrict__ binbase,
                       unsigned long long *__restrict__ nexthist, unsigned long long *status ,
                       unsigned *__restrict__ ticket, unsigned long long *__restrict__ hiflag)
{ constexpr int ITEMS = os64_tile<IW>::ITEMS, TILE = os64_tile<IW>::TILE;
  extern __shared__ __align__(16) unsigned char smem_raw[];
  unsigned long long *tile = reinterpret_cast<unsigned long long *>(smem_raw);
  unsigned *wcount = reinterpret_cast<unsigned *>(smem_raw + (size_t) TILE*IW);
  unsigned *bexcl  = wcount + SORT_WARPS*256;
  unsigned *nhist  = bexcl + 256;
  unsigned *wtot   = nhist + 256;
  unsigned long long *gbase = reinterpret_cast<unsigned long long *>(wtot + 8);
  __shared__ unsigned tile_s;
  __shared__ __align__(8) unsigned long long tbar;

  int tid = threadIdx.x, lane = tid & 31, w = tid >> 5;
  if (tid == 0)
    { unsigned t = atomicAdd(ticket,1u);
      tile_s = t;
      long long t0 = (long long) t * TILE, rm = n - t0;
      unsigned nb = ((unsigned) (rm < TILE ? rm : TILE) * IW + 15u) & ~15u;
      mbar_init(&tbar,1);
      tma_load_1d(tile,reinterpret_cast<const unsigned char *>(in) + t0*IW,nb,&tbar);
    }
  for (int i = tid; i < SORT_WARPS*256; i += SORT_THREADS) wcount[i] = 0;
  if (tid < 256) nhist[tid] = 0;
  __syncthreads();
  const unsigned tileid = tile_s;
  long long tile0 = (long long) tileid * TILE;
  long long rem = n - tile0;
  int cnt = rem < TILE ? (int) rem : TILE;

  unsigned long long r[ITEMS], hi_or = 0;
  unsigned rank[ITEMS];
  int base = w*(32*ITEMS);
  unsigned *myc = wcount + w*256;
  mbar_wait(&tbar,0);
#pragma unroll
  for (int it = 0; it < ITEMS; it++)
    { int idx = base + it*32 + lane;
      bool valid = idx < cnt;
      unsigned d = 0;
      if (valid)
        { if (IW == 16)
            { rec128 v = ld_rec(reinterpret_cast<const rec128 *>(tile) + idx);
              r[it] = v.lo;
              hi_or |= v.hi;
            }
          else
            r[it] = tile[idx];
          d = (unsigned) (r[it] >> dsh) & 0xff;
        }
      unsigned peers = match_digit(d,valid);
      int leader = valid ? __ffs(peers)-1 : lane;
      unsigned b = 0;
      if (valid && lane == leader)
        { b = myc[d];
          myc[d] = b + __popc(peers);
        }
      b = __shfl_sync(0xffffffffu,b,leader);
      rank[it] = b + __popc(peers & lanemask_lt());
      if (next_dsh >= 0 && valid) atomicAdd(&nhist[(unsigned) (r[it] >> next_dsh) & 0xff],1u);
      __syncwarp();
    }
  if (IW == 16 && hi_or) atomicOr(hiflag,hi_or);
  __syncthreads();

  unsigned c = 0, inc = 0;
  unsigned long long *mine = status + (unsigned long long) tileid*256 + tid;
  if (tid < 256)
    { unsigned sum = 0;
#pragma unroll
      for (int ww = 0; ww < SORT_WARPS; ww++)
        { unsigned t = wcount[ww*256+tid];
          wcount[ww*256+tid] = sum;
          sum += t;
        }
      c = sum;
      if (tileid == 0)
        atomicExch(mine,ST_INC | c);
      else
        atomicExch(mine,ST_AGG | c);
      inc = warp_incl_scan(c,lane);
      if (lane == 31) wtot[w] = inc;
    }
  __syncthreads();
  if (tid < 256)
    { unsigned pre = 0;
      for (int i = 0; i < w; i++) pre += wtot[i];
      bexcl[tid] = pre + inc - c;
    }
  __syncthreads();

#pragma unroll
  for (int it = 0; it < ITEMS; it++)
    { int idx = base + it*32 + lane;
      if (idx < cnt)
        { unsigned d = (unsigned) (r[it] >> dsh) & 0xff;
          tile[bexcl[d] + myc[d] + rank[it]] = r[it];
        }
    }
  if (tid < 256)
    { volatile unsigned long long *stt = status;
      unsigned long long excl = 0;
      for (long long t = (long long) tileid - 1; t >= 0; )
        { unsigned long long v[4];
#pragma unroll
          for (int q = 0; q < 4; q++)
            v[q] = (t - q >= 0) ? stt[(unsigned long long) (t - q)*256 + tid] : ST_INC;
          bool done = false;
#pragma unroll
          for (int q = 0; q < 4; q++)
            { if (done || (v[q] >> 62) == 0) break;
              excl += v[q] & ST_MASK;
              t -= 1;
              if (v[q] & ST_INC) done = true;
            }
          if (done) break;
        }
      if (tileid != 0) atomicExch(mine,ST_INC | (excl + c));
      gbase[tid] = binbase[tid] + excl - bexcl[tid];
      if (next_dsh >= 0 && nhist[tid]) atomicAdd(&nexthist[tid],(unsigned long long) nhist[tid]);
    }
  __syncthreads();

  for (int p = tid; p < cnt; p += SORT_THREADS)
    { unsigned long long v = tile[p];
      unsigned long long o = gbase[(unsigned) (v >> dsh) & 0xff] + p;
      if (OW == 8)
        reinterpret_cast<unsigned long long *>(out)[o] = v;
      else
        { rec128 R; R.lo = v; R.hi = 0;
          st_rec(reinterpret_cast<rec128 *>(out) + o,R);
        }
    }
}

template <int IW, int OW>
static int onesweep64_pass(const void *in, void *out, long long n, int dsh, int next_dsh, const unsigned long long *binbase,
                           unsigned long long *nexthist, unsigned long long *status, unsigned *ticket,
                           unsigned long long *hiflag, cudaStream_t st)
{ typedef os64_tile<IW> T;
  static bool attr_set = false;
  if (!attr_set)
    { CUDA_TRY(cudaFuncSetAttribute(sort_onesweep64_kernel<IW,OW>,cudaFuncAttributeMaxDynamicSharedMemorySize,(int) T::SMEM));
      attr_set = true;
    }
  int ntiles = (int) ((n + T::TILE - 1) / T::TILE);
  CUDA_TRY(cudaMemsetAsync(status,0,256ull*ntiles*8,st));
  sort_onesweep64_kernel<IW,OW><<<ntiles,SORT_THREADS,T::SMEM,st>>>(in,out,n,dsh,next_dsh,binbase,nexthist,status,ticket,hiflag);
  fgb_count_launch(1);
  return FGB_OK;
}

extern "C" int fgb_sort_seeds64_device(void *d_a, void *d_b, long long n, int bit_lo, int bit_hi,
                                       void *d_tmp, long long tmp_bytes, unsigned long long *d_flag, void *stream)
{ cudaStream_t st = (cudaStream_t) stream;
  if (n < 0 || bit_lo < 0 || bit_hi > 64 || bit_lo > bit_hi) return FGB_ERR_ARG;
  if (n >= 0xffffffffll) return FGB_ERR_LIMIT;
  CUDA_TRY(cudaMemsetAsync(d_flag,0,8,st));
  if (n <= 1 || bit_lo == bit_hi) return FGB_OK;
  if (tmp_bytes < fgb_sort128_tmp_bytes(n)) return FGB_ERR_ARG;
  if (bit_hi - bit_lo <= 8)
    { int inb = 0;
      int rc = fgb_sort128_bits_device(d_a,d_b,n,bit_lo,bit_hi,d_tmp,tmp_bytes,&inb,stream);
      if (rc) return rc;
      if (inb) CUDA_TRY(cudaMemcpyAsync(d_a,d_b,sizeof(rec128)*n,cudaMemcpyDeviceToDevice,st));
      return FGB_OK;
    }

  int ntiles = (int) ((n + SORT_TILE - 1) / SORT_TILE);
  unsigned long long *status = (unsigned long long *) d_tmp;
  unsigned long long *hist[2] = { status + 256ull*ntiles, status + 256ull*ntiles + 256 };
  unsigned long long *binbase = status + 256ull*ntiles + 512;
  unsigned *ticket = (unsigned *) (binbase + 256);
  unsigned char *half[2] = { (unsigned char *) d_b, (unsigned char *) d_b + ((8*n + 15) & ~15ll) };

  CUDA_TRY(cudaMemsetAsync(hist[0],0,256*8,st));
  { int nb = ntiles < 1184 ? ntiles : 1184;
    sort_ghist_kernel<<<nb,SORT_THREADS,0,st>>>((const rec128 *) d_a,n,bit_lo,hist[0]);
    fgb_count_launch(1);
  }
  int cur = 0, rc = FGB_OK;
  for (int p = 0, b = bit_lo; b < bit_hi && rc == FGB_OK; p++, b += 8)
    { const int nd = (b+8 < bit_hi) ? b+8 : -1;
      sort_bins_kernel<<<1,256,0,st>>>(hist[cur],binbase,hist[cur^1],ticket);
      fgb_count_launch(1);
      if (p == 0)
        rc = onesweep64_pass<16,8>(d_a,half[0],n,b,nd,binbase,hist[cur^1],status,ticket,d_flag,st);
      else if (nd >= 0)
        rc = onesweep64_pass<8,8>(half[(p-1)&1],half[p&1],n,b,nd,binbase,hist[cur^1],status,ticket,d_flag,st);
      else
        rc = onesweep64_pass<8,16>(half[(p-1)&1],d_a,n,b,nd,binbase,hist[cur^1],status,ticket,d_flag,st);
      cur ^= 1;
    }
  if (rc) return rc;
  CUDA_TRY(cudaGetLastError());
  return FGB_OK;
}


#define BK_THREADS SORT_THREADS
#define BK_ITEMS   8
#define BK_CAP     (BK_THREADS*BK_ITEMS)
#define BK_WARPS   SORT_WARPS
#define BK_SPAN    4
#define BK_SUBBITS 10
#define BK_NSUB    (BK_SPAN << BK_SUBBITS)
#define BK_MAXSUB  32

__global__ void kmer_bins_kernel(const rec128 *__restrict__ tab, long long n, int binshift, unsigned long long base,
                                 unsigned *__restrict__ bin_start, long long nbins)
{ long long i = (long long) blockIdx.x * blockDim.x + threadIdx.x;
  if (i > n) return;
  long long lo = (i == 0) ? -1 : (long long) ((tab[i-1].hi >> binshift) - base);
  long long hi = (i == n) ? nbins : (long long) ((tab[i].hi >> binshift) - base);
  if (hi > nbins) hi = nbins;
  for (long long p = lo+1; p <= hi; p++) bin_start[p] = (unsigned) i;
}

extern "C" int fgb_kmer_bins_device(const void *d_tab, long long n, int binshift, unsigned *d_bins, void *stream)
{ int nb = (int) ((n + 1 + 255) / 256);
  kmer_bins_kernel<<<nb,256,0,(cudaStream_t) stream>>>((const rec128 *) d_tab,n,binshift,0ull,d_bins,65536ll);
  fgb_count_launch(1);
  CUDA_TRY(cudaGetLastError());
  return FGB_OK;
}


__global__ void __launch_bounds__(BK_THREADS,2)
kmer_bucket_sort_kernel(const rec128 *__restrict__ in, rec128 *__restrict__ out,
                        const uint2 *__restrict__ groups , int binshift)
{ extern __shared__ __align__(16) unsigned char smem_raw[];
  rec128   *tile   = reinterpret_cast<rec128 *>(smem_raw);
  unsigned *cnt    = reinterpret_cast<unsigned *>(tile + BK_CAP);
  unsigned *bexcl  = cnt + BK_NSUB + 32;
  unsigned *wtot   = bexcl + 256;
  __shared__ __align__(8) unsigned long long tbar;

  const int tid = threadIdx.x, lane = tid & 31, w = tid >> 5;
  const uint2 g = groups[blockIdx.x];
  const int count = (int) g.y;
  if (tid == 0)
    { mbar_init(&tbar,1);
      tma_load_1d(tile,in + g.x,(unsigned) count * 16u,&tbar);
    }
  for (int i = tid; i <= BK_NSUB; i += BK_THREADS) cnt[i] = 0;
  __syncthreads();
  mbar_wait(&tbar,0);

  rec128   r[BK_ITEMS];
  unsigned sub[BK_ITEMS], off[BK_ITEMS];
  const int base = w*(32*BK_ITEMS);
  const unsigned b0 = (unsigned) (tile[0].hi >> binshift);
  const int subshift = binshift - BK_SUBBITS;
#pragma unroll
  for (int it = 0; it < BK_ITEMS; it++)
    { int idx = base + it*32 + lane;
      if (idx < count)
        { r[it] = ld_rec(tile + idx);
          sub[it] = ((((unsigned) (r[it].hi >> binshift)) - b0) << BK_SUBBITS) | ((unsigned) (r[it].hi >> subshift) & ((1u << BK_SUBBITS)-1));
          off[it] = atomicAdd(&cnt[sub[it]],1u);
        }
    }
  __syncthreads();
  bool big = false;
  { unsigned v[8], sum = 0;
#pragma unroll
    for (int i = 0; i < 8; i++) { v[i] = cnt[8*tid+i]; big |= (v[i] > BK_MAXSUB); sum += v[i]; }
    unsigned inc = warp_incl_scan(sum,lane);
    if (lane == 31) wtot[w] = inc;
    __syncthreads();
    unsigned pre = inc - sum;
    for (int i = 0; i < w; i++) pre += wtot[i];
#pragma unroll
    for (int i = 0; i < 8; i++) { cnt[8*tid+i] = pre; pre += v[i]; }
    if (tid == BK_THREADS-1) cnt[BK_NSUB] = pre;
  }
  big = __syncthreads_or(big);

  if (!big)
    {
#pragma unroll
      for (int it = 0; it < BK_ITEMS; it++)
        { int idx = base + it*32 + lane;
          if (idx < count) st_rec(tile + (cnt[sub[it]] + off[it]),r[it]);
        }
      __syncthreads();
      for (int p = tid; p < count; p += BK_THREADS)
        { rec128 R = ld_rec(tile + p);
          unsigned sb = ((((unsigned) (R.hi >> binshift)) - b0) << BK_SUBBITS) | ((unsigned) (R.hi >> subshift) & ((1u << BK_SUBBITS)-1));
          int s = (int) cnt[sb], e = (int) cnt[sb+1], rank = 0;
          for (int q = s; q < e; q++)
            { rec128 Q = ld_rec(tile + q);
              bool less = (Q.hi < R.hi) || (Q.hi == R.hi && (Q.lo < R.lo || (Q.lo == R.lo && q < p)));
              rank += less;
            }
          st_rec(out + (g.x + s + rank),R);
        }
      return;
    }

  unsigned *wcount = cnt;
  unsigned *myc = wcount + w*256;
  unsigned rank[BK_ITEMS];
  __syncthreads();
#pragma unroll
  for (int i = 0; i < 8; i++) myc[i*32 + lane] = 0;
  __syncwarp();
  for (int byte = 0; byte < 16; byte++)
    {
#pragma unroll
      for (int it = 0; it < BK_ITEMS; it++)
        { int idx = base + it*32 + lane;
          bool valid = idx < count;
          unsigned d = valid ? rec_byte(r[it],byte) : 0;
          unsigned peers = match_digit(d,valid);
          int leader = valid ? __ffs(peers)-1 : lane;
          unsigned b = 0;
          if (valid && lane == leader)
            { b = myc[d];
              myc[d] = b + __popc(peers);
            }
          b = __shfl_sync(0xffffffffu,b,leader);
          rank[it] = b + __popc(peers & lanemask_lt());
          __syncwarp();
        }
      __syncthreads();
      unsigned c = 0, inc = 0;
      if (tid < 256)
        { unsigned sum = 0;
#pragma unroll
          for (int ww = 0; ww < BK_WARPS; ww++)
            { unsigned t = wcount[ww*256+tid];
              wcount[ww*256+tid] = sum;
              sum += t;
            }
          c = sum;
          inc = warp_incl_scan(c,lane);
          if (lane == 31) wtot[w] = inc;
        }
      __syncthreads();
      if (tid < 256)
        { unsigned pre = 0;
          for (int i = 0; i < w; i++) pre += wtot[i];
          bexcl[tid] = pre + inc - c;
        }
      __syncthreads();
#pragma unroll
      for (int it = 0; it < BK_ITEMS; it++)
        { int idx = base + it*32 + lane;
          if (idx < count)
            { unsigned d = rec_byte(r[it],byte);
              st_rec(tile + (bexcl[d] + myc[d] + rank[it]),r[it]);
            }
        }
      __syncthreads();
      if (byte + 1 < 16)
        {
#pragma unroll
          for (int it = 0; it < BK_ITEMS; it++)
            { int idx = base + it*32 + lane;
              if (idx < count) r[it] = ld_rec(tile + idx);
            }
#pragma unroll
          for (int i = 0; i < 8; i++) myc[i*32 + lane] = 0;
          __syncwarp();
        }
    }
  for (int p = tid; p < count; p += BK_THREADS)
    st_rec(out + (g.x + p),ld_rec(tile + p));
}

__global__ void kmer_copy_segments_kernel(const rec128 *__restrict__ src, rec128 *__restrict__ dst,
                                          const unsigned *__restrict__ sfrom, const unsigned *__restrict__ dfrom,
                                          const unsigned *__restrict__ pre, int nseg, long long total)
{ for (long long i = (long long) blockIdx.x * blockDim.x + threadIdx.x; i < total;
       i += (long long) gridDim.x * blockDim.x)
    { int lo = 0, hi = nseg;
      while (hi - lo > 1) { int md = (lo+hi) >> 1; if (pre[md] <= i) lo = md; else hi = md; }
      unsigned o = (unsigned) (i - pre[lo]);
      st_rec(dst + (dfrom[lo] + o),ld_rec(src + (sfrom[lo] + o)));
    }
}

static const size_t BUCKET_SMEM = BK_CAP*sizeof(rec128) + (BK_NSUB + 32 + 256 + BK_WARPS)*sizeof(unsigned);



extern "C" int fgb_kmer_sort_range_device(void *d_a, void *d_b, long long n, unsigned plo, unsigned phi,
                                          void *d_tmp, long long tmp_bytes, int *result_in_b, void *stream)
{ cudaStream_t st = (cudaStream_t) stream;
  *result_in_b = 0;
  if (n <= 1) return FGB_OK;
  if (n >= 0xffffffffll) return FGB_ERR_LIMIT;
  if (phi <= plo || phi > (1u << 24)) return FGB_ERR_ARG;
  long long maxbins = 65536, target = 1536;
  if (getenv("FGB_KSORT_BIN_TARGET") != NULL) target = atoll(getenv("FGB_KSORT_BIN_TARGET"));
  if (target < 1) target = 1;
  while (maxbins < (1ll << 24) && n / maxbins > target) maxbins <<= 1;
  int sh = 0;
  while ((long long) ((((unsigned long long) (phi - 1) >> sh) - ((unsigned long long) plo >> sh))) >= maxbins) sh += 1;
  const int binshift = 40 + sh;
  const unsigned long long base = (unsigned long long) plo >> sh;
  const long long nbins = (long long) (((unsigned long long) (phi - 1) >> sh) - base) + 1;
  int inb = 0;
  int rc = fgb_sort128_bits_device(d_a,d_b,n,64 + binshift,128,d_tmp,tmp_bytes,&inb,st);
  if (rc) return rc;
  rec128 *src = (rec128 *) (inb ? d_b : d_a), *dst = (rec128 *) (inb ? d_a : d_b);

  static bool attr_set = false;
  if (!attr_set)
    { CUDA_TRY(cudaFuncSetAttribute(kmer_bucket_sort_kernel,cudaFuncAttributeMaxDynamicSharedMemorySize,
                                    (int) BUCKET_SMEM));
      attr_set = true;
    }

  unsigned *d_bins = NULL;
  CUDA_TRY(fgb_dmalloc((void **) &d_bins,sizeof(unsigned)*(size_t) (nbins+1),st));
  { int nb = (int) ((n + 1 + 255) / 256);
    kmer_bins_kernel<<<nb,256,0,st>>>(src,n,binshift,base,d_bins,nbins);
    fgb_count_launch(1);
  }
  std::vector<unsigned> bins((size_t) nbins + 1);
  CUDA_TRY(cudaMemcpyAsync(bins.data(),d_bins,sizeof(unsigned)*(size_t) (nbins+1),cudaMemcpyDeviceToHost,st));
  CUDA_TRY(cudaStreamSynchronize(st));

  std::vector<uint2> groups;
  std::vector<unsigned> ofrom, opre;
  unsigned ototal = 0;
  { unsigned gs = bins[0], gc = 0; long long gp = 0;
    for (long long p = 0; p < nbins; p++)
      { unsigned len = bins[p+1] - bins[p];
        if (len == 0) continue;
        if (len > BK_CAP)
          { if (gc) { groups.push_back(make_uint2(gs,gc)); gc = 0; }
            ofrom.push_back(bins[p]); opre.push_back(ototal); ototal += len;
            continue;
          }
        if (gc != 0 && (gc + len > BK_CAP || p - gp >= BK_SPAN))
          { groups.push_back(make_uint2(gs,gc)); gc = 0; }
        if (gc == 0) { gs = bins[p]; gp = p; }
        gc += len;
      }
    if (gc) groups.push_back(make_uint2(gs,gc));
  }

  uint2 *d_groups = NULL;
  if (!groups.empty())
    { CUDA_TRY(fgb_dmalloc((void **) &d_groups,sizeof(uint2)*groups.size(),st));
      CUDA_TRY(cudaMemcpyAsync(d_groups,groups.data(),sizeof(uint2)*groups.size(),cudaMemcpyHostToDevice,st));
      kmer_bucket_sort_kernel<<<(unsigned) groups.size(),BK_THREADS,BUCKET_SMEM,st>>>(src,dst,d_groups,binshift);
      fgb_count_launch(1);
      CUDA_TRY(cudaGetLastError());
    }
  if (ototal > 0)
    { int nseg = (int) ofrom.size();
      opre.push_back(ototal);
      std::vector<unsigned> cfrom(opre.begin(),opre.end()-1);
      rec128 *d_c1 = NULL, *d_c2 = NULL; void *d_ctmp = NULL; unsigned *d_seg = NULL;
      long long ctb = fgb_sort128_tmp_bytes(ototal);
      CUDA_TRY(fgb_dmalloc((void **) &d_c1,sizeof(rec128)*((size_t) ototal+1),st));
      CUDA_TRY(fgb_dmalloc((void **) &d_c2,sizeof(rec128)*((size_t) ototal+1),st));
      CUDA_TRY(fgb_dmalloc(&d_ctmp,ctb,st));
      CUDA_TRY(fgb_dmalloc((void **) &d_seg,sizeof(unsigned)*(3*(size_t) nseg+1),st));
      CUDA_TRY(cudaMemcpyAsync(d_seg,ofrom.data(),sizeof(unsigned)*nseg,cudaMemcpyHostToDevice,st));
      CUDA_TRY(cudaMemcpyAsync(d_seg+nseg,cfrom.data(),sizeof(unsigned)*nseg,cudaMemcpyHostToDevice,st));
      CUDA_TRY(cudaMemcpyAsync(d_seg+2*nseg,opre.data(),sizeof(unsigned)*(nseg+1),cudaMemcpyHostToDevice,st));
      int nb = (int) ((ototal + 255) / 256); if (nb > 4736) nb = 4736;
      kmer_copy_segments_kernel<<<nb,256,0,st>>>(src,d_c1,d_seg,d_seg+nseg,d_seg+2*nseg,nseg,ototal);
      int cinb = 0;
      rc = fgb_sort128_device(d_c1,d_c2,ototal,0,16,d_ctmp,ctb,&cinb,st);
      if (rc) return rc;
      kmer_copy_segments_kernel<<<nb,256,0,st>>>(cinb ? d_c2 : d_c1,dst,d_seg+nseg,d_seg,d_seg+2*nseg,nseg,ototal);
      fgb_count_launch(2);
      CUDA_TRY(cudaGetLastError());
      CUDA_TRY(cudaStreamSynchronize(st));
      fgb_dfree(d_c1,st); fgb_dfree(d_c2,st); fgb_dfree(d_ctmp,st); fgb_dfree(d_seg,st);
    }
  CUDA_TRY(cudaStreamSynchronize(st));
  fgb_dfree(d_bins,st); if (d_groups) fgb_dfree(d_groups,st);
  *result_in_b = inb ^ 1;
  return FGB_OK;
}

extern "C" int fgb_kmer_sort_device(void *d_a, void *d_b, long long n, void *d_tmp, long long tmp_bytes,
                                    int *result_in_b, void *stream)
{ return fgb_kmer_sort_range_device(d_a,d_b,n,0,1u << 24,d_tmp,tmp_bytes,result_in_b,stream); }


#define SCAN_THREADS 1024
#define SCAN_ITEMS   8
#define SCAN_TILE    (SCAN_THREADS*SCAN_ITEMS)

__global__ void __launch_bounds__(SCAN_THREADS)
scan_reduce_kernel(const unsigned *__restrict__ data, long long n, unsigned long long *__restrict__ sums)
{ __shared__ unsigned long long ws[32];
  long long t0 = (long long) blockIdx.x * SCAN_TILE;
  unsigned long long s = 0;
  for (int i = 0; i < SCAN_ITEMS; i++)
    { long long idx = t0 + i*SCAN_THREADS + threadIdx.x;
      if (idx < n) s += data[idx];
    }
  for (int o = 16; o > 0; o >>= 1) s += __shfl_down_sync(0xffffffffu,s,o);
  if ((threadIdx.x & 31) == 0) ws[threadIdx.x >> 5] = s;
  __syncthreads();
  if (threadIdx.x < 32)
    { s = ws[threadIdx.x];
      for (int o = 16; o > 0; o >>= 1) s += __shfl_down_sync(0xffffffffu,s,o);
      if (threadIdx.x == 0) sums[blockIdx.x] = s;
    }
}

__global__ void __launch_bounds__(1024)
scan_sums_kernel(unsigned long long *__restrict__ sums, int nb, unsigned long long *__restrict__ total)
{ __shared__ unsigned long long ws[32];
  __shared__ unsigned long long carry_s;
  int tid = threadIdx.x, lane = tid & 31, w = tid >> 5;
  if (tid == 0) carry_s = 0;
  __syncthreads();
  for (int base = 0; base < nb; base += 1024)
    { int i = base + tid;
      unsigned long long v = (i < nb) ? sums[i] : 0, inc = v;
      for (int o = 1; o < 32; o <<= 1)
        { unsigned long long t = __shfl_up_sync(0xffffffffu,inc,o);
          if (lane >= o) inc += t;
        }
      if (lane == 31) ws[w] = inc;
      __syncthreads();
      if (w == 0)
        { unsigned long long s = ws[lane], si = s;
          for (int o = 1; o < 32; o <<= 1)
            { unsigned long long t = __shfl_up_sync(0xffffffffu,si,o);
              if (lane >= o) si += t;
            }
          ws[lane] = si - s;
        }
      __syncthreads();
      unsigned long long ex = carry_s + ws[w] + inc - v;
      if (i < nb) sums[i] = ex;
      __syncthreads();
      if (tid == 1023) carry_s = ex + v;
      __syncthreads();
    }
  if (tid == 0 && total != NULL) *total = carry_s;
}

__global__ void __launch_bounds__(SCAN_THREADS)
scan_down_kernel(unsigned *__restrict__ data, long long n, const unsigned long long *__restrict__ sums)
{ __shared__ unsigned ws[32];
  int tid = threadIdx.x, lane = tid & 31, w = tid >> 5;
  long long t0 = (long long) blockIdx.x * SCAN_TILE + (long long) tid * SCAN_ITEMS;
  unsigned v[SCAN_ITEMS], s = 0;
#pragma unroll
  for (int i = 0; i < SCAN_ITEMS; i++)
    { v[i] = (t0 + i < n) ? data[t0+i] : 0;
      s += v[i];
    }
  unsigned inc = warp_incl_scan(s,lane);
  if (lane == 31) ws[w] = inc;
  __syncthreads();
  if (w == 0)
    { unsigned x = ws[lane];
      unsigned xi = warp_incl_scan(x,lane);
      ws[lane] = xi - x;
    }
  __syncthreads();
  unsigned ex = (unsigned) sums[blockIdx.x] + ws[w] + inc - s;
#pragma unroll
  for (int i = 0; i < SCAN_ITEMS; i++)
    { if (t0 + i < n) data[t0+i] = ex;
      ex += v[i];
    }
}

long long fgb_dev_scan_tmp_bytes(long long n)
{ long long nb = (n + SCAN_TILE - 1) / SCAN_TILE;
  if (nb < 1) nb = 1;
  return nb * 8 + 64;
}


int fgb_dev_exclusive_scan_u32(unsigned *d_data, long long n, unsigned long long *d_total,
                               void *d_tmp, long long tmp_bytes, cudaStream_t st)
{ if (n <= 0)
    { if (d_total) CUDA_TRY(cudaMemsetAsync(d_total,0,8,st));
      return FGB_OK;
    }
  if (tmp_bytes < fgb_dev_scan_tmp_bytes(n)) return FGB_ERR_ARG;
  int nb = (int) ((n + SCAN_TILE - 1) / SCAN_TILE);
  unsigned long long *sums = (unsigned long long *) d_tmp;
  scan_reduce_kernel<<<nb,SCAN_THREADS,0,st>>>(d_data,n,sums);
  scan_sums_kernel<<<1,1024,0,st>>>(sums,nb,d_total);
  scan_down_kernel<<<nb,SCAN_THREADS,0,st>>>(d_data,n,sums);
  fgb_count_launch(3);
  CUDA_TRY(cudaGetLastError());
  return FGB_OK;
}
```

Baseline: 3.753.

## Scatter syncmers directly into fine key bins, skipping partition radix pass

The syncmer scan now counts k-mers per fine prefix bin with atomics. A second scan scatters each record straight into its bin, so the k-mer sort no longer needs the initial radix partition pass or the separate bin histogram. The bin boundaries are computed on the host from the fine-bin starts, and the per-bin bucket sort then runs directly. This trades a memory pass for atomic-contended scattered writes and non-deterministic order within bins, and the old path stays available behind an environment variable.

```diff
diff --git a/fastga_b200/csrc/api.cu b/fastga_b200/csrc/api.cu
--- a/fastga_b200/csrc/api.cu
+++ b/fastga_b200/csrc/api.cu
@@ -32,6 +32,19 @@
                             const int *d_crank, const int *d_tile_contig, const int *d_tile_start,
                             int ntiles, unsigned *d_tile_offset, void *d_records, unsigned plo,
                             unsigned phi, void *stream);
+int fgb_kmer_bin_shift(long long n, unsigned plo, unsigned phi);
+int fgb_syncmer_bin_count_device(const void *d_seq, const long long *d_clen, const long long *d_woff,
+                                 const int *d_crank, const int *d_tile_contig, const int *d_tile_start,
+                                 int ntiles, unsigned long long *d_buck1024, unsigned *d_bin_start, long long nf,
+                                 int fsh, unsigned long long *d_total, void *d_tmp, long long tmp_bytes,
+                                 unsigned plo, unsigned phi, void *stream);
+int fgb_syncmer_scatter_device(const void *d_seq, const long long *d_clen, const long long *d_woff,
+                               const int *d_crank, const int *d_tile_contig, const int *d_tile_start,
+                               int ntiles, const unsigned *d_bin_start, unsigned *d_cursor, long long nf, int fsh,
+                               long long n, void *d_records, unsigned *d_bad, unsigned plo, unsigned phi,
+                               void *stream);
+int fgb_kmer_sort_fine_binned_device(void *d_a, void *d_b, long long n, unsigned plo, unsigned phi,
+                                     const unsigned *fstart, long long nf, int fsh, int *result_in_b, void *stream);
 int fgb_kix_index_device(const void *d_tab, long long n, unsigned *d_pstart, unsigned char *d_adj, void *stream);
 int fgb_ktab_export_device(const void *d_tab, long long n, int pbytes, int cbytes,
                            const long long *d_part_first, int nparts, void *d_out, void *stream);
@@ -269,66 +282,107 @@
   return gix_build_range(g,plo,phi,out,stream);
 }
 
+struct fine_bins
+{ int fsh = 0;
+  long long nf = 0;
+  std::vector<unsigned> start;
+};
+
 static int gix_scan(const fgb_genome *g, const unsigned char *mask, unsigned plo, unsigned phi_flags,
-                    rec128 **d_recs, long long *n_out, long long *nrev, unsigned long long *buck1024, cudaStream_t st)
+                    rec128 **d_recs, long long *n_out, long long *nrev, unsigned long long *buck1024,
+                    fine_bins *fb, cudaStream_t st)
 { int T = fgb_sc_tile();
   std::vector<int> tc, ts;
+  long long npos = 0;
   for (int c = 0; c < g->ncontig; c++)
     if (g->clen[c] >= 12 && g->boff[c] >= 0 && (mask == NULL || mask[c]))
-      for (long long t0 = 0; t0 + 12 <= g->clen[c]; t0 += T)
-        { tc.push_back(c); ts.push_back((int) t0); }
+      { npos += g->clen[c] - 11;
+        for (long long t0 = 0; t0 + 12 <= g->clen[c]; t0 += T)
+          { tc.push_back(c); ts.push_back((int) t0); }
+      }
   int ntiles = (int) tc.size();
   int *d_tc = NULL, *d_ts = NULL; unsigned *d_cnt = NULL;
   u64 *d_buck = NULL, *d_total = NULL; void *d_tmp = NULL;
+  unsigned *d_fb = NULL, bad = 0;
+  long long nf = 0;
   rec128 *d_a = NULL;
   long long tmpb = fgb_dev_scan_tmp_bytes(ntiles);
   int rc = FGB_OK;
   u64 total = 0, rdropped = 0;
+  if (fb)
+    { const unsigned phi = phi_flags & ~GIX_FWD_ONLY;
+      const unsigned bhi = phi > plo ? phi : plo + 1;
+      fb->fsh = fgb_kmer_bin_shift(2*npos,plo,bhi);
+      fb->nf = nf = (long long) ((((unsigned long long) (bhi - 1)) >> fb->fsh) - ((unsigned long long) plo >> fb->fsh)) + 1;
+      tmpb = fgb_dev_scan_tmp_bytes(nf);
+    }
 #define GS_TRY(call) do { if ((call) != cudaSuccess) { rc = FGB_ERR_CUDA; goto done; } } while (0)
   GS_TRY(fgb_dmalloc((void **) &d_tc,sizeof(int)*(ntiles+1),st));
   GS_TRY(fgb_dmalloc((void **) &d_ts,sizeof(int)*(ntiles+1),st));
-  GS_TRY(fgb_dmalloc((void **) &d_cnt,sizeof(unsigned)*(ntiles+1),st));
+  if (fb) GS_TRY(fgb_dmalloc((void **) &d_fb,sizeof(unsigned)*(2*nf+1),st));
+  else    GS_TRY(fgb_dmalloc((void **) &d_cnt,sizeof(unsigned)*(ntiles+1),st));
   GS_TRY(fgb_dmalloc((void **) &d_buck,8*1025,st));
   GS_TRY(fgb_dmalloc((void **) &d_total,8,st));
   GS_TRY(fgb_dmalloc((void **) &d_tmp,tmpb,st));
   GS_TRY(cudaMemcpyAsync(d_tc,tc.data(),sizeof(int)*ntiles,cudaMemcpyHostToDevice,st));
   GS_TRY(cudaMemcpyAsync(d_ts,ts.data(),sizeof(int)*ntiles,cudaMemcpyHostToDevice,st));
   { stage_timer t(&g_timings.scan_ms,st);
-    rc = fgb_syncmer_count_device(g->d_seq,g->d_clen,g->d_woff,g->d_crank,d_tc,d_ts,ntiles,d_cnt,
-                                  d_buck,d_total,d_tmp,tmpb,plo,phi_flags,st);
+    if (fb)
+      rc = fgb_syncmer_bin_count_device(g->d_seq,g->d_clen,g->d_woff,g->d_crank,d_tc,d_ts,ntiles,d_buck,d_fb,nf,
+                                        fb->fsh,d_total,d_tmp,tmpb,plo,phi_flags,st);
+    else
+      rc = fgb_syncmer_count_device(g->d_seq,g->d_clen,g->d_woff,g->d_crank,d_tc,d_ts,ntiles,d_cnt,
+                                    d_buck,d_total,d_tmp,tmpb,plo,phi_flags,st);
     if (rc) goto done;
     GS_TRY(cudaMemcpyAsync(&total,d_total,8,cudaMemcpyDeviceToHost,st));
     if (buck1024) GS_TRY(cudaMemcpyAsync(buck1024,d_buck,8*1024,cudaMemcpyDeviceToHost,st));
     GS_TRY(cudaMemcpyAsync(&rdropped,d_buck + 1024,8,cudaMemcpyDeviceToHost,st));
+    if (fb)
+      { fb->start.resize((size_t) nf + 1);
+        GS_TRY(cudaMemcpyAsync(fb->start.data(),d_fb,sizeof(unsigned)*nf,cudaMemcpyDeviceToHost,st));
+      }
     GS_TRY(cudaStreamSynchronize(st));
   }
   if (total >= 0xfffffff0ull) { rc = FGB_ERR_LIMIT; goto done; }
   GS_TRY(fgb_dmalloc((void **) &d_a,sizeof(rec128)*(total+1),st));
   { stage_timer t(&g_timings.scan_ms,st);
-    rc = fgb_syncmer_emit_device(g->d_seq,g->d_clen,g->d_woff,g->d_crank,d_tc,d_ts,ntiles,d_cnt,d_a,plo,phi_flags,st);
+    if (fb)
+      { rc = fgb_syncmer_scatter_device(g->d_seq,g->d_clen,g->d_woff,g->d_crank,d_tc,d_ts,ntiles,d_fb,d_fb + nf,nf,
+                                        fb->fsh,(long long) total,d_a,d_fb + 2*nf,plo,phi_flags,st);
+        if (!rc && cudaMemcpyAsync(&bad,d_fb + 2*nf,4,cudaMemcpyDeviceToHost,st) != cudaSuccess) rc = FGB_ERR_CUDA;
+      }
+    else
+      rc = fgb_syncmer_emit_device(g->d_seq,g->d_clen,g->d_woff,g->d_crank,d_tc,d_ts,ntiles,d_cnt,d_a,plo,phi_flags,st);
   }
   if (rc == FGB_OK && cudaStreamSynchronize(st) != cudaSuccess) rc = FGB_ERR_CUDA;
+  if (rc == FGB_OK && bad) rc = FGB_ERR_OVERFLOW;
+  if (rc == FGB_OK && fb) fb->start[nf] = (unsigned) total;
 done:
 #undef GS_TRY
-  fgb_dfree(d_tc,st); fgb_dfree(d_ts,st); fgb_dfree(d_cnt,st); fgb_dfree(d_buck,st); fgb_dfree(d_total,st); fgb_dfree(d_tmp,st);
+  fgb_dfree(d_tc,st); fgb_dfree(d_ts,st); fgb_dfree(d_cnt,st); fgb_dfree(d_fb,st); fgb_dfree(d_buck,st);
+  fgb_dfree(d_total,st); fgb_dfree(d_tmp,st);
   if (rc) { fgb_dfree(d_a,st); return rc; }
   *d_recs = d_a; *n_out = (long long) total; *nrev = (long long) rdropped;
   return FGB_OK;
 }
 
-static int gix_finish(fgb_gix *x, rec128 *d_a, long long n, unsigned plo, unsigned phi, cudaStream_t st, bool index = true)
+static int gix_finish(fgb_gix *x, rec128 *d_a, long long n, unsigned plo, unsigned phi, const fine_bins *fb,
+                      cudaStream_t st, bool index = true)
 { rec128 *d_b = NULL; void *d_stmp = NULL;
   long long stmpb = fgb_sort128_tmp_bytes(n);
   int rc = FGB_OK, inb = 0;
   x->n = n;
   if (fgb_dmalloc((void **) &d_b,sizeof(rec128)*(n+1),st) != cudaSuccess ||
-      fgb_dmalloc((void **) &d_stmp,stmpb,st) != cudaSuccess ||
+      (!fb && fgb_dmalloc((void **) &d_stmp,stmpb,st) != cudaSuccess) ||
       (index && fgb_dmalloc((void **) &x->d_pstart,sizeof(unsigned)*((1<<24)+1+8),st) != cudaSuccess) ||
       (index && fgb_dmalloc((void **) &x->d_adj,(size_t) n + 32,st) != cudaSuccess))
     rc = FGB_ERR_CUDA;
   if (!rc)
     { stage_timer t(&g_timings.ksort_ms,st);
-      rc = fgb_kmer_sort_range_device(d_a,d_b,n,plo,phi,d_stmp,stmpb,&inb,st);
+      if (fb)
+        rc = fgb_kmer_sort_fine_binned_device(d_a,d_b,n,plo,phi,fb->start.data(),fb->nf,fb->fsh,&inb,st);
+      else
+        rc = fgb_kmer_sort_range_device(d_a,d_b,n,plo,phi,d_stmp,stmpb,&inb,st);
     }
   if (!rc)
     { x->d_tab = inb ? d_b : d_a;
@@ -353,8 +407,10 @@
   x->ncontig = g->ncontig;
   x->fwd_only = (phi_flags & GIX_FWD_ONLY) ? 1 : 0;
   rec128 *d_a = NULL; long long n = 0, nrev = 0;
-  int rc = gix_scan(g,NULL,plo,phi_flags,&d_a,&n,&nrev,x->buck1024,st);
-  if (!rc) { x->n_both = n + nrev; rc = gix_finish(x,d_a,n,plo,phi,st,index); }
+  const char *part_env = getenv("FGB_KSORT_PARTITION");
+  fine_bins fb, *pfb = (part_env != NULL && atoi(part_env) != 0) ? NULL : &fb;
+  int rc = gix_scan(g,NULL,plo,phi_flags,&d_a,&n,&nrev,x->buck1024,pfb,st);
+  if (!rc) { x->n_both = n + nrev; rc = gix_finish(x,d_a,n,plo,phi,pfb,st,index); }
   if (rc) { fgb_gix_free(x); return rc; }
   *out = x;
   return FGB_OK;
@@ -368,7 +424,7 @@
 extern "C" int fgb_kmers_scan(const fgb_genome *g, const unsigned char *mask, int fwd_only,
                               void **d_recs, long long *n, void *stream)
 { rec128 *d = NULL; long long nrev = 0;
-  int rc = gix_scan(g,mask,0u,(1u << 24) | (fwd_only ? GIX_FWD_ONLY : 0u),&d,n,&nrev,NULL,(cudaStream_t) stream);
+  int rc = gix_scan(g,mask,0u,(1u << 24) | (fwd_only ? GIX_FWD_ONLY : 0u),&d,n,&nrev,NULL,NULL,(cudaStream_t) stream);
   if (rc) return rc;
   *d_recs = d;
   return FGB_OK;
@@ -407,7 +463,7 @@
   int rc = FGB_OK;
   if (fgb_dmalloc((void **) &d_a,sizeof(rec128)*(n+1),st) != cudaSuccess) rc = FGB_ERR_CUDA;
   if (!rc && n > 0 && cudaMemcpyAsync(d_a,d_recs,sizeof(rec128)*n,cudaMemcpyDeviceToDevice,st) != cudaSuccess) rc = FGB_ERR_CUDA;
-  if (!rc) rc = gix_finish(x,d_a,n,plo,phi,st); else fgb_dfree(d_a,st);
+  if (!rc) rc = gix_finish(x,d_a,n,plo,phi,NULL,st); else fgb_dfree(d_a,st);
   if (rc) { fgb_gix_free(x); return rc; }
   *out = x;
   return FGB_OK;
diff --git a/fastga_b200/csrc/gix.cu b/fastga_b200/csrc/gix.cu
--- a/fastga_b200/csrc/gix.cu
+++ b/fastga_b200/csrc/gix.cu
@@ -144,17 +144,17 @@
   return sel;
 }
 
-template<int EMIT> __global__ void __launch_bounds__(SC_THREADS)
-syncmer_kernel(const u64 *__restrict__ seq, const long long *__restrict__ clen,
-               const long long *__restrict__ woff, const int *__restrict__ crank,
-               const int *__restrict__ tile_contig, const int *__restrict__ tile_start,
-               unsigned *__restrict__ tile_count,
-               unsigned long long *__restrict__ buck1024,
-               rec128 *__restrict__ out, unsigned plo, unsigned phi_flags)
+template<int EMIT, bool BINNED> static __device__ __forceinline__ void
+syncmer_body(const u64 *__restrict__ seq, const long long *__restrict__ clen,
+             const long long *__restrict__ woff, const int *__restrict__ crank,
+             const int *__restrict__ tile_contig, const int *__restrict__ tile_start,
+             unsigned *__restrict__ tile_count, unsigned long long *__restrict__ buck1024,
+             rec128 *__restrict__ out, unsigned plo, unsigned phi_flags,
+             unsigned *__restrict__ bincur, int fsh, unsigned nlim)
 { __shared__ u64 sw[SC_WORDS+1];
   __shared__ unsigned char tn[256], tc[256];
   __shared__ unsigned wsum[SC_THREADS/32];
-  __shared__ unsigned hist[1024];
+  __shared__ unsigned hist[EMIT == 0 ? 1024 : 1];
 
   const unsigned phi = phi_flags & 0x7fffffffu;
   const bool fwd_only = (phi_flags >> 31) != 0;
@@ -211,18 +211,52 @@
   unsigned cnt = __popc(fmask) + __popc(rmask);
 
   int lane = tid & 31, wp = tid >> 5;
-  unsigned inc = cnt;
+  unsigned pre = 0, tot = 0, inc = cnt;
+  if (!BINNED)
+    {
 #pragma unroll
-  for (int o = 1; o < 32; o <<= 1)
-    { unsigned t = __shfl_up_sync(0xffffffffu,inc,o);
-      if (lane >= o) inc += t;
-    }
-  if (lane == 31) wsum[wp] = inc;
-  __syncthreads();
-  unsigned pre = 0, tot = 0;
-  for (int i = 0; i < SC_THREADS/32; i++)
-    { if (i < wp) pre += wsum[i];
-      tot += wsum[i];
+      for (int o = 1; o < 32; o <<= 1)
+        { unsigned t = __shfl_up_sync(0xffffffffu,inc,o);
+          if (lane >= o) inc += t;
+        }
+      if (lane == 31) wsum[wp] = inc;
+      __syncthreads();
+      for (int i = 0; i < SC_THREADS/32; i++)
+        { if (i < wp) pre += wsum[i];
+          tot += wsum[i];
+        }
+    }
+  const unsigned cr = (unsigned) crank[c];
+
+  if (BINNED)
+    {
+      const unsigned fbase = plo >> fsh;
+      unsigned fm = fmask, rm = rmask;
+      while (fm | rm)
+        { rec128 r;
+          r.lo = 0;
+          if (fm)
+            { int i = __ffs(fm)-1;
+              fm &= fm-1;
+              r.hi = rev2(sm_bases64(sw,sb+i));
+              if (EMIT)
+                r.lo = (rev2(sm_bases64(sw,sb+i+32)) & 0xffff000000000000ull) | ((u64) cr << 32) | (unsigned) (p+i);
+            }
+          else
+            { int i = __ffs(rm)-1;
+              rm &= rm-1;
+              u64 e0 = sm_bases64(sw,sb+i-28), e1 = sm_bases64(sw,sb+i+4) & 0xffffull;
+              r.hi = ~((e1 << 48) | (e0 >> 16));
+              r.lo = ((~e0 & 0xffffull) << 48) | ((u64) (cr | 0x8000u) << 32) | (unsigned) (p+i+12);
+            }
+          const unsigned b = (unsigned) (r.hi >> (40 + fsh)) - fbase;
+          if (EMIT == 0)
+            atomicAdd(&bincur[b],1u);
+          else
+            { const unsigned s = atomicAdd(&bincur[b],1u);
+              if (s < nlim) st_rec(out + s,r);
+            }
+        }
     }
 
   if (EMIT == 0)
@@ -249,12 +283,12 @@
         { rdropped = __reduce_add_sync(0xffffffffu,rdropped);
           if (lane == 0 && rdropped) atomicAdd(&buck1024[1024],(unsigned long long) rdropped);
         }
-      if (tid == 0) tile_count[blockIdx.x] = tot;
+      if (!BINNED && tid == 0) tile_count[blockIdx.x] = tot;
       return;
     }
+  if (BINNED) return;
 
   long long o = (long long) tile_count[blockIdx.x] + pre + inc - cnt;
-  unsigned cr = (unsigned) crank[c];
   unsigned m = fmask | rmask;
   while (m)
     { int i = __ffs(m)-1;
@@ -279,6 +313,39 @@
           o += 1;
         }
     }
+}
+
+template<int EMIT> __global__ void __launch_bounds__(SC_THREADS)
+syncmer_kernel(const u64 *__restrict__ seq, const long long *__restrict__ clen,
+               const long long *__restrict__ woff, const int *__restrict__ crank,
+               const int *__restrict__ tile_contig, const int *__restrict__ tile_start,
+               unsigned *__restrict__ tile_count,
+               unsigned long long *__restrict__ buck1024,
+               rec128 *__restrict__ out, unsigned plo, unsigned phi_flags)
+{ syncmer_body<EMIT,false>(seq,clen,woff,crank,tile_contig,tile_start,tile_count,buck1024,out,plo,phi_flags,NULL,0,0); }
+
+__global__ void __launch_bounds__(SC_THREADS)
+syncmer_bin_count_kernel(const u64 *__restrict__ seq, const long long *__restrict__ clen,
+                         const long long *__restrict__ woff, const int *__restrict__ crank,
+                         const int *__restrict__ tile_contig, const int *__restrict__ tile_start,
+                         unsigned long long *__restrict__ buck1024, unsigned plo, unsigned phi_flags,
+                         unsigned *__restrict__ bin_count, int fsh)
+{ syncmer_body<0,true>(seq,clen,woff,crank,tile_contig,tile_start,NULL,buck1024,NULL,plo,phi_flags,bin_count,fsh,0); }
+
+__global__ void __launch_bounds__(SC_THREADS)
+syncmer_scatter_kernel(const u64 *__restrict__ seq, const long long *__restrict__ clen,
+                       const long long *__restrict__ woff, const int *__restrict__ crank,
+                       const int *__restrict__ tile_contig, const int *__restrict__ tile_start,
+                       rec128 *__restrict__ out, unsigned n, unsigned plo, unsigned phi_flags,
+                       unsigned *__restrict__ bin_cursor, int fsh)
+{ syncmer_body<1,true>(seq,clen,woff,crank,tile_contig,tile_start,NULL,NULL,out,plo,phi_flags,bin_cursor,fsh,n); }
+
+__global__ void kmer_scatter_check_kernel(const unsigned *__restrict__ cursor, const unsigned *__restrict__ start,
+                                          long long nf, unsigned n, unsigned *__restrict__ bad)
+{ long long f = (long long) blockIdx.x * blockDim.x + threadIdx.x;
+  if (f >= nf) return;
+  unsigned end = (f + 1 < nf) ? start[f+1] : n;
+  if (cursor[f] != end) *bad = 1;
 }
 
 
@@ -431,6 +498,50 @@
   return FGB_OK;
 }
 
+extern "C" int fgb_syncmer_bin_count_device(const void *d_seq, const long long *d_clen,
+                                            const long long *d_woff, const int *d_crank,
+                                            const int *d_tile_contig, const int *d_tile_start, int ntiles,
+                                            unsigned long long *d_buck1024, unsigned *d_bin_start, long long nf,
+                                            int fsh, unsigned long long *d_total, void *d_tmp, long long tmp_bytes,
+                                            unsigned plo, unsigned phi, void *stream)
+{ cudaStream_t st = (cudaStream_t) stream;
+  int rc = init_tables();
+  if (rc) return rc;
+  CUDA_TRY(cudaMemsetAsync(d_buck1024,0,1025*8,st));
+  CUDA_TRY(cudaMemsetAsync(d_bin_start,0,sizeof(unsigned)*nf,st));
+  if (ntiles > 0)
+    { syncmer_bin_count_kernel<<<ntiles,SC_THREADS,0,st>>>((const u64 *) d_seq,d_clen,d_woff,d_crank,
+                                                           d_tile_contig,d_tile_start,d_buck1024,plo,phi,
+                                                           d_bin_start,fsh);
+      fgb_count_launch(1);
+    }
+  CUDA_TRY(cudaGetLastError());
+  return fgb_dev_exclusive_scan_u32(d_bin_start,nf,d_total,d_tmp,tmp_bytes,st);
+}
+
+extern "C" int fgb_syncmer_scatter_device(const void *d_seq, const long long *d_clen,
+                                          const long long *d_woff, const int *d_crank,
+                                          const int *d_tile_contig, const int *d_tile_start, int ntiles,
+                                          const unsigned *d_bin_start, unsigned *d_cursor, long long nf, int fsh,
+                                          long long n, void *d_records, unsigned *d_bad, unsigned plo,
+                                          unsigned phi, void *stream)
+{ cudaStream_t st = (cudaStream_t) stream;
+  CUDA_TRY(cudaMemcpyAsync(d_cursor,d_bin_start,sizeof(unsigned)*nf,cudaMemcpyDeviceToDevice,st));
+  CUDA_TRY(cudaMemsetAsync(d_bad,0,sizeof(unsigned),st));
+  if (ntiles > 0)
+    { syncmer_scatter_kernel<<<ntiles,SC_THREADS,0,st>>>((const u64 *) d_seq,d_clen,d_woff,d_crank,
+                                                         d_tile_contig,d_tile_start,(rec128 *) d_records,
+                                                         (unsigned) n,plo,phi,d_cursor,fsh);
+      fgb_count_launch(1);
+    }
+  if (nf > 0)
+    { kmer_scatter_check_kernel<<<(unsigned) ((nf + 255) / 256),256,0,st>>>(d_cursor,d_bin_start,nf,(unsigned) n,d_bad);
+      fgb_count_launch(1);
+    }
+  CUDA_TRY(cudaGetLastError());
+  return FGB_OK;
+}
+
 __global__ void kix_ends_kernel(const rec128 *__restrict__ tab, long long n, unsigned *__restrict__ pstart)
 { long long x = (long long) blockIdx.x * blockDim.x + threadIdx.x;
   if (x > (1ll << 24)) return;
diff --git a/fastga_b200/csrc/sort128.cu b/fastga_b200/csrc/sort128.cu
--- a/fastga_b200/csrc/sort128.cu
+++ b/fastga_b200/csrc/sort128.cu
@@ -514,7 +514,8 @@
 
 __global__ void __launch_bounds__(BK_THREADS,2)
 kmer_bucket_sort_kernel(const rec128 *__restrict__ in, rec128 *__restrict__ out,
-                        const uint2 *__restrict__ groups , int binshift)
+                        const uint4 *__restrict__ groups ,
+                        int binshift)
 { extern __shared__ __align__(16) unsigned char smem_raw[];
   rec128   *tile   = reinterpret_cast<rec128 *>(smem_raw);
   unsigned *cnt    = reinterpret_cast<unsigned *>(tile + BK_CAP);
@@ -523,7 +524,7 @@
   __shared__ __align__(8) unsigned long long tbar;
 
   const int tid = threadIdx.x, lane = tid & 31, w = tid >> 5;
-  const uint2 g = groups[blockIdx.x];
+  const uint4 g = groups[blockIdx.x];
   const int count = (int) g.y;
   if (tid == 0)
     { mbar_init(&tbar,1);
@@ -536,7 +537,7 @@
   rec128   r[BK_ITEMS];
   unsigned sub[BK_ITEMS], off[BK_ITEMS];
   const int base = w*(32*BK_ITEMS);
-  const unsigned b0 = (unsigned) (tile[0].hi >> binshift);
+  const unsigned b0 = g.z;
   const int subshift = binshift - BK_SUBBITS;
 #pragma unroll
   for (int it = 0; it < BK_ITEMS; it++)
@@ -670,29 +671,21 @@
 
 static const size_t BUCKET_SMEM = BK_CAP*sizeof(rec128) + (BK_NSUB + 32 + 256 + BK_WARPS)*sizeof(unsigned);
 
-
-
-extern "C" int fgb_kmer_sort_range_device(void *d_a, void *d_b, long long n, unsigned plo, unsigned phi,
-                                          void *d_tmp, long long tmp_bytes, int *result_in_b, void *stream)
-{ cudaStream_t st = (cudaStream_t) stream;
-  *result_in_b = 0;
-  if (n <= 1) return FGB_OK;
-  if (n >= 0xffffffffll) return FGB_ERR_LIMIT;
-  if (phi <= plo || phi > (1u << 24)) return FGB_ERR_ARG;
-  long long maxbins = 65536, target = 1536;
+extern "C" int fgb_kmer_bin_shift(long long n, unsigned plo, unsigned phi)
+{ long long maxbins = 65536, target = 1536;
   if (getenv("FGB_KSORT_BIN_TARGET") != NULL) target = atoll(getenv("FGB_KSORT_BIN_TARGET"));
   if (target < 1) target = 1;
   while (maxbins < (1ll << 24) && n / maxbins > target) maxbins <<= 1;
   int sh = 0;
   while ((long long) ((((unsigned long long) (phi - 1) >> sh) - ((unsigned long long) plo >> sh))) >= maxbins) sh += 1;
-  const int binshift = 40 + sh;
-  const unsigned long long base = (unsigned long long) plo >> sh;
-  const long long nbins = (long long) (((unsigned long long) (phi - 1) >> sh) - base) + 1;
-  int inb = 0;
-  int rc = fgb_sort128_bits_device(d_a,d_b,n,64 + binshift,128,d_tmp,tmp_bytes,&inb,st);
-  if (rc) return rc;
-  rec128 *src = (rec128 *) (inb ? d_b : d_a), *dst = (rec128 *) (inb ? d_a : d_b);
-
+  return sh;
+}
+
+static int kmer_sort_binned(const rec128 *src, rec128 *dst, const unsigned *bins, long long nbins, int sh,
+                            unsigned plo, cudaStream_t st)
+{ const int binshift = 40 + sh;
+  const unsigned base = plo >> sh;
+  int rc = FGB_OK;
   static bool attr_set = false;
   if (!attr_set)
     { CUDA_TRY(cudaFuncSetAttribute(kmer_bucket_sort_kernel,cudaFuncAttributeMaxDynamicSharedMemorySize,
@@ -700,17 +693,7 @@
       attr_set = true;
     }
 
-  unsigned *d_bins = NULL;
-  CUDA_TRY(fgb_dmalloc((void **) &d_bins,sizeof(unsigned)*(size_t) (nbins+1),st));
-  { int nb = (int) ((n + 1 + 255) / 256);
-    kmer_bins_kernel<<<nb,256,0,st>>>(src,n,binshift,base,d_bins,nbins);
-    fgb_count_launch(1);
-  }
-  std::vector<unsigned> bins((size_t) nbins + 1);
-  CUDA_TRY(cudaMemcpyAsync(bins.data(),d_bins,sizeof(unsigned)*(size_t) (nbins+1),cudaMemcpyDeviceToHost,st));
-  CUDA_TRY(cudaStreamSynchronize(st));
-
-  std::vector<uint2> groups;
+  std::vector<uint4> groups;
   std::vector<unsigned> ofrom, opre;
   unsigned ototal = 0;
   { unsigned gs = bins[0], gc = 0; long long gp = 0;
@@ -718,22 +701,22 @@
       { unsigned len = bins[p+1] - bins[p];
         if (len == 0) continue;
         if (len > BK_CAP)
-          { if (gc) { groups.push_back(make_uint2(gs,gc)); gc = 0; }
+          { if (gc) { groups.push_back(make_uint4(gs,gc,base + (unsigned) gp,0)); gc = 0; }
             ofrom.push_back(bins[p]); opre.push_back(ototal); ototal += len;
             continue;
           }
         if (gc != 0 && (gc + len > BK_CAP || p - gp >= BK_SPAN))
-          { groups.push_back(make_uint2(gs,gc)); gc = 0; }
+          { groups.push_back(make_uint4(gs,gc,base + (unsigned) gp,0)); gc = 0; }
         if (gc == 0) { gs = bins[p]; gp = p; }
         gc += len;
       }
-    if (gc) groups.push_back(make_uint2(gs,gc));
+    if (gc) groups.push_back(make_uint4(gs,gc,base + (unsigned) gp,0));
   }
 
-  uint2 *d_groups = NULL;
+  uint4 *d_groups = NULL;
   if (!groups.empty())
-    { CUDA_TRY(fgb_dmalloc((void **) &d_groups,sizeof(uint2)*groups.size(),st));
-      CUDA_TRY(cudaMemcpyAsync(d_groups,groups.data(),sizeof(uint2)*groups.size(),cudaMemcpyHostToDevice,st));
+    { CUDA_TRY(fgb_dmalloc((void **) &d_groups,sizeof(uint4)*groups.size(),st));
+      CUDA_TRY(cudaMemcpyAsync(d_groups,groups.data(),sizeof(uint4)*groups.size(),cudaMemcpyHostToDevice,st));
       kmer_bucket_sort_kernel<<<(unsigned) groups.size(),BK_THREADS,BUCKET_SMEM,st>>>(src,dst,d_groups,binshift);
       fgb_count_launch(1);
       CUDA_TRY(cudaGetLastError());
@@ -763,8 +746,61 @@
       fgb_dfree(d_c1,st); fgb_dfree(d_c2,st); fgb_dfree(d_ctmp,st); fgb_dfree(d_seg,st);
     }
   CUDA_TRY(cudaStreamSynchronize(st));
-  fgb_dfree(d_bins,st); if (d_groups) fgb_dfree(d_groups,st);
+  if (d_groups) fgb_dfree(d_groups,st);
+  return FGB_OK;
+}
+
+extern "C" int fgb_kmer_sort_range_device(void *d_a, void *d_b, long long n, unsigned plo, unsigned phi,
+                                          void *d_tmp, long long tmp_bytes, int *result_in_b, void *stream)
+{ cudaStream_t st = (cudaStream_t) stream;
+  *result_in_b = 0;
+  if (n <= 1) return FGB_OK;
+  if (n >= 0xffffffffll) return FGB_ERR_LIMIT;
+  if (phi <= plo || phi > (1u << 24)) return FGB_ERR_ARG;
+  const int sh = fgb_kmer_bin_shift(n,plo,phi);
+  const int binshift = 40 + sh;
+  const unsigned long long base = (unsigned long long) plo >> sh;
+  const long long nbins = (long long) (((unsigned long long) (phi - 1) >> sh) - base) + 1;
+  int inb = 0;
+  int rc = fgb_sort128_bits_device(d_a,d_b,n,64 + binshift,128,d_tmp,tmp_bytes,&inb,st);
+  if (rc) return rc;
+  rec128 *src = (rec128 *) (inb ? d_b : d_a), *dst = (rec128 *) (inb ? d_a : d_b);
+
+  unsigned *d_bins = NULL;
+  CUDA_TRY(fgb_dmalloc((void **) &d_bins,sizeof(unsigned)*(size_t) (nbins+1),st));
+  { int nb = (int) ((n + 1 + 255) / 256);
+    kmer_bins_kernel<<<nb,256,0,st>>>(src,n,binshift,base,d_bins,nbins);
+    fgb_count_launch(1);
+  }
+  std::vector<unsigned> bins((size_t) nbins + 1);
+  CUDA_TRY(cudaMemcpyAsync(bins.data(),d_bins,sizeof(unsigned)*(size_t) (nbins+1),cudaMemcpyDeviceToHost,st));
+  CUDA_TRY(cudaStreamSynchronize(st));
+  fgb_dfree(d_bins,st);
+  rc = kmer_sort_binned(src,dst,bins.data(),nbins,sh,plo,st);
+  if (rc) return rc;
   *result_in_b = inb ^ 1;
+  return FGB_OK;
+}
+
+extern "C" int fgb_kmer_sort_fine_binned_device(void *d_a, void *d_b, long long n, unsigned plo, unsigned phi,
+                                                const unsigned *fstart, long long nf, int fsh, int *result_in_b,
+                                                void *stream)
+{ *result_in_b = 0;
+  if (n <= 1) return FGB_OK;
+  if (n >= 0xffffffffll) return FGB_ERR_LIMIT;
+  if (phi <= plo || phi > (1u << 24)) return FGB_ERR_ARG;
+  const int sh = fgb_kmer_bin_shift(n,plo,phi);
+  if (sh < fsh || (long long) fstart[nf] != n) return FGB_ERR_ARG;
+  const unsigned long long base = (unsigned long long) plo >> sh, fbase = (unsigned long long) plo >> fsh;
+  const long long nbins = (long long) (((unsigned long long) (phi - 1) >> sh) - base) + 1;
+  std::vector<unsigned> bins((size_t) nbins + 1);
+  for (long long p = 0; p <= nbins; p++)
+    { long long f = (long long) ((base + p) << (sh - fsh)) - (long long) fbase;
+      bins[p] = fstart[f < 0 ? 0 : (f > nf ? nf : f)];
+    }
+  int rc = kmer_sort_binned((const rec128 *) d_a,(rec128 *) d_b,bins.data(),nbins,sh,plo,(cudaStream_t) stream);
+  if (rc) return rc;
+  *result_in_b = 1;
   return FGB_OK;
 }
 
diff --git a/profiles/kmer_build_bench.py b/profiles/kmer_build_bench.py
--- /dev/null
+++ b/profiles/kmer_build_bench.py
@@ -0,0 +1,116 @@
+#!/usr/bin/env python
+import argparse
+import hashlib
+import json
+import os
+import subprocess
+import sys
+
+import numpy as np
+
+ROOT = os.path.dirname(os.path.dirname(os.path.abspath(__file__)))
+sys.path.insert(0, ROOT)
+
+PEAK_GBS = 3350.0
+BYTES = {"scatter": 48, "partition": 144}
+
+
+def gpu_info():
+    try:
+        out = subprocess.run(["nvidia-smi", "--query-gpu=name,power.limit,clocks.max.sm", "--format=csv,noheader"],
+                             stdout=subprocess.PIPE, text=True, check=True).stdout.strip().split("\n")[0]
+        name, power, mhz = [s.strip() for s in out.split(",")]
+        return {"name": name, "power_limit": power, "sm_max_clock": mhz}
+    except Exception as ex:
+        return {"error": str(ex)[:200]}
+
+
+def set_path(path):
+    if path == "partition":
+        os.environ["FGB_KSORT_PARTITION"] = "1"
+    else:
+        os.environ.pop("FGB_KSORT_PARTITION", None)
+
+
+def main():
+    ap = argparse.ArgumentParser()
+    ap.add_argument("--reps", type=int, default=15)
+    ap.add_argument("--warmup", type=int, default=2)
+    args = ap.parse_args()
+
+    import torch
+    import bench
+    from fastga_b200 import formats, lib
+
+    A, B = bench.workload(1)
+    gA, gB = formats.genome_from_arrays(A), formats.genome_from_arrays(B)
+    dA, dB = lib.DeviceGenome(gA), lib.DeviceGenome(gB)
+
+    def build(path):
+        set_path(path)
+        lib.timings_reset()
+        xA, xB = lib.DeviceGix.build_forward(dA), lib.DeviceGix.build(dB)
+        t = lib.timings_get()
+        return (xA, xB), t["scan_ms"], t["ksort_ms"]
+
+    paths = ("scatter", "partition")
+    ms = {p: {"scan": [], "ksort": []} for p in paths}
+    for i in range(args.warmup + args.reps):
+        for p in paths:
+            xs, scan, ksort = build(p)
+            for x in xs:
+                x.close()
+            if i >= args.warmup:
+                ms[p]["scan"].append(scan)
+                ms[p]["ksort"].append(ksort)
+
+    digests, n = {}, None
+    for p in paths:
+        xs, _, _ = build(p)
+        digests[p] = [hashlib.md5(a.tobytes()).hexdigest() for x in xs for a in x.download()]
+        n = [x.n for x in xs]
+        for x in xs:
+            x.close()
+    identical = digests["scatter"] == digests["partition"]
+
+    kernels = {}
+    for p in paths:
+        for x in build(p)[0]:
+            x.close()
+        with torch.profiler.profile(activities=[torch.profiler.ProfilerActivity.CUDA]) as prof:
+            xs, _, _ = build(p)
+            torch.cuda.synchronize()
+        for x in xs:
+            x.close()
+        k = {}
+        for e in prof.key_averages():
+            t = getattr(e, "device_time_total", None)
+            if t is None:
+                t = e.cuda_time_total
+            if t > 0:
+                k[e.key.split("(")[0][:60]] = round(t / 1000.0, 4)
+        kernels[p] = dict(sorted(k.items(), key=lambda kv: -kv[1]))
+    set_path("scatter")
+    torch.cuda.synchronize()
+
+    nrec = sum(n)
+
+    def summary(p):
+        scan, ksort = np.array(ms[p]["scan"]), np.array(ms[p]["ksort"])
+        tot = scan + ksort
+        med = float(np.median(tot))
+        gbs = nrec * BYTES[p] / med / 1e6
+        return {"scan_plus_ksort_ms_median": med, "min_max": [float(tot.min()), float(tot.max())],
+                "scan_ms_median": float(np.median(scan)), "ksort_ms_median": float(np.median(ksort)),
+                "reps": len(tot), "bytes_per_record": BYTES[p], "bytes": nrec * BYTES[p], "GB_s": gbs,
+                "frac_of_3350_GB_s": gbs / PEAK_GBS, "kernel_ms_profiled_build": kernels[p]}
+
+    line = {"what": "k-mer tables of the bench pair (bench.py workload, N = 1): A forward-only + B both strands",
+            "gpu": gpu_info(), "records": n, "scatter": summary("scatter"), "partition": summary("partition"),
+            "tables_pstart_buck_byte_identical": identical}
+    line["speedup"] = line["partition"]["scan_plus_ksort_ms_median"] / line["scatter"]["scan_plus_ksort_ms_median"]
+    print(json.dumps(line))
+
+
+if __name__ == "__main__":
+    main()
```

New measurement: 3.947 (median of 6 runs). 1.05x the previous value.
